# Ced3-han/PepFlowww

Measured on AMD Instinct MI355X. Metric: residues x denoise-steps / s, higher is better.
Workload: dtype f32 (fp32 storage and accumulation; matrix products as 3 x f16 split MFMA, ~22-bit operands); 1 GPU; cfg4/GPU: B=64 x 128-residue synthetic pockets (112 ctx + 16 gen) per GPU; per_gpu_batch=64, residues=128, global_batch=64, parallelism=batch-shard x1, hipgraph=True, precision=fp32

## Files before the change

pepflowww_amd/csrc/common.h:

```cpp
#pragma once
#include <hip/hip_runtime.h>

static inline int pf_cu_count() {
    static int cache[64] = {0};
    int dev = 0, c = 256;
    if (hipGetDevice(&dev) != hipSuccess) return 256;
    if (dev >= 0 && dev < 64 && cache[dev] > 0) return cache[dev];
    if (hipDeviceGetAttribute(&c, hipDeviceAttributeMultiprocessorCount, dev) != hipSuccess || c <= 0) c = 256;
    if (dev >= 0 && dev < 64) cache[dev] = c;
    return c;
}
#include <stdint.h>

#define PF_WAVE 64

typedef float f32x4 __attribute__((ext_vector_type(4)));

__device__ __forceinline__ f32x4 mfma16(float a, float b, f32x4 c) {
    return __builtin_amdgcn_mfma_f32_16x16x4f32(a, b, c, 0, 0, 0);
}

__device__ __forceinline__ void lds_barrier() {
    asm volatile("s_waitcnt lgkmcnt(0)" ::: "memory");
    __builtin_amdgcn_s_barrier();
    asm volatile("" ::: "memory");
}

template <int CTRL, int BANK = 0xF>
__device__ __forceinline__ float dpp_mov(float old, float v) {
    return __int_as_float(__builtin_amdgcn_update_dpp(__float_as_int(old), __float_as_int(v), CTRL, 0xF, BANK, false));
}
__device__ __forceinline__ float lane_xor1(float v) { return dpp_mov<0xB1>(v, v); }
__device__ __forceinline__ float lane_xor2(float v) { return dpp_mov<0x4E>(v, v); }
__device__ __forceinline__ float lane_xor4(float v) {
    float t = dpp_mov<0x104, 0x5>(v, v);
    return dpp_mov<0x114, 0xA>(t, v);
}
__device__ __forceinline__ float lane_xor8(float v) { return dpp_mov<0x128>(v, v); }
template <int OFF> __device__ __forceinline__ float lane_xor(float v) {
    if constexpr (OFF == 1) return lane_xor1(v);
    else if constexpr (OFF == 2) return lane_xor2(v);
    else if constexpr (OFF == 4) return lane_xor4(v);
    else return lane_xor8(v);
}
__device__ __forceinline__ float sum_xor16(float v) {
    auto r = __builtin_amdgcn_permlane16_swap(__float_as_uint(v), __float_as_uint(v), false, false);
    return __uint_as_float(r[0]) + __uint_as_float(r[1]);
}
__device__ __forceinline__ float sum_xor32(float v) {
    auto r = __builtin_amdgcn_permlane32_swap(__float_as_uint(v), __float_as_uint(v), false, false);
    return __uint_as_float(r[0]) + __uint_as_float(r[1]);
}
__device__ __forceinline__ float max_xor16(float v) {
    auto r = __builtin_amdgcn_permlane16_swap(__float_as_uint(v), __float_as_uint(v), false, false);
    return fmaxf(__uint_as_float(r[0]), __uint_as_float(r[1]));
}
__device__ __forceinline__ float max_xor32(float v) {
    auto r = __builtin_amdgcn_permlane32_swap(__float_as_uint(v), __float_as_uint(v), false, false);
    return fmaxf(__uint_as_float(r[0]), __uint_as_float(r[1]));
}
__device__ __forceinline__ bool pf_rows_all_masked(const int* __restrict__ key_end, int L, int m0, int n, int M) {
    if (!key_end) return false;
    const int mend = m0 + n < M ? m0 + n : M;
    int m = m0;
    while (m < mend) {
        const int b = m / L, i = m - b * L;
        if (i < key_end[b]) return false;
        m = (b + 1) * L;
    }
    return true;
}
__device__ __forceinline__ float row16_sum(float v) {
    v += lane_xor8(v); v += lane_xor4(v); v += lane_xor2(v); v += lane_xor1(v);
    return v;
}
__device__ __forceinline__ float row16_max(float v) {
    v = fmaxf(v, lane_xor8(v)); v = fmaxf(v, lane_xor4(v)); v = fmaxf(v, lane_xor2(v)); v = fmaxf(v, lane_xor1(v));
    return v;
}
__device__ __forceinline__ float wave_sum(float v) { return sum_xor32(sum_xor16(row16_sum(v))); }
__device__ __forceinline__ float wave_max(float v) { return max_xor32(max_xor16(row16_max(v))); }

__device__ __forceinline__ float keep_if(bool ok, float v) { return __uint_as_float(__float_as_uint(v) & (ok ? 0xffffffffu : 0u)); }
__device__ __forceinline__ float4 keep_if(bool ok, const float4& v) {
    const unsigned m = ok ? 0xffffffffu : 0u;
    return make_float4(__uint_as_float(__float_as_uint(v.x) & m), __uint_as_float(__float_as_uint(v.y) & m),
                       __uint_as_float(__float_as_uint(v.z) & m), __uint_as_float(__float_as_uint(v.w) & m));
}

template <int MT, int NT>
__device__ __forceinline__ void mfma_slice(const float4 (&a)[MT], const float4 (&b)[NT], f32x4 (&acc)[MT][NT]) {
#pragma unroll
    for (int mt = 0; mt < MT; ++mt)
#pragma unroll
        for (int nt = 0; nt < NT; ++nt) {
            acc[mt][nt] = mfma16(a[mt].x, b[nt].x, acc[mt][nt]);
            acc[mt][nt] = mfma16(a[mt].y, b[nt].y, acc[mt][nt]);
            acc[mt][nt] = mfma16(a[mt].z, b[nt].z, acc[mt][nt]);
            acc[mt][nt] = mfma16(a[mt].w, b[nt].w, acc[mt][nt]);
        }
}

template <int NT, int PF_DEPTH = 4>
struct BStream {
    const float* wrow[NT];
    bool wok[NT];
    float4 ring[PF_DEPTH][NT];
    int nslices;

    __device__ __forceinline__ void init(const float* __restrict__ W, int ldw, int n0, int n_valid, int K) {
        const int lane = threadIdx.x & 63;
        const int r = lane & 15, g = lane >> 4;
        nslices = K >> 4;
#pragma unroll
        for (int nt = 0; nt < NT; ++nt) {
            const int n = n0 + 16 * nt + r;
            wok[nt] = n < n_valid;
            wrow[nt] = W + (size_t)(wok[nt] ? n : 0) * ldw + 4 * g;
        }
    }
    __device__ __forceinline__ void load(int slot_static, int slice, float4 (&dst)[NT]) {
        (void)slot_static;
#pragma unroll
        for (int nt = 0; nt < NT; ++nt)
            dst[nt] = *reinterpret_cast<const float4*>(wrow[nt] + 16 * slice);
    }
    __device__ __forceinline__ void prefetch() {
#pragma unroll
        for (int d = 0; d < PF_DEPTH; ++d)
            if (d < nslices) load(d, d, ring[d]);
    }
};

template <int MT, int NT, int PF_DEPTH>
__device__ __forceinline__ void gemm_ldsA_stream(const float* __restrict__ A_lds, int lda, BStream<NT, PF_DEPTH>& bs,
                                                 f32x4 (&acc)[MT][NT], int slice0, int count) {
    const int lane = threadIdx.x & 63;
    const float* arow = A_lds + (lane & 15) * lda + 4 * (lane >> 4);
    const int ns = bs.nslices;
    for (int base = 0; base < count; base += PF_DEPTH) {
#pragma unroll
        for (int u = 0; u < PF_DEPTH; ++u) {
            if (base + u < count) {
                const int sl = slice0 + base + u;
                float4 a[MT];
#pragma unroll
                for (int mt = 0; mt < MT; ++mt)
                    a[mt] = *reinterpret_cast<const float4*>(arow + mt * 16 * lda + 16 * (base + u));
                mfma_slice<MT, NT>(a, bs.ring[u], acc);
                if (sl + PF_DEPTH < ns) bs.load(u, sl + PF_DEPTH, bs.ring[u]);
            }
        }
    }
}

template <int MT, int NT>
__device__ __forceinline__ void gemm_ldsA_glbB(const float* __restrict__ A_lds, int lda,
                                               const float* __restrict__ W, int ldw, int n0, int n_valid,
                                               int K, f32x4 (&acc)[MT][NT]) {
    BStream<NT> bs;
    bs.init(W, ldw, n0, n_valid, K);
    bs.prefetch();
    gemm_ldsA_stream<MT, NT, 4>(A_lds, lda, bs, acc, 0, bs.nslices);
}

typedef _Float16 half8 __attribute__((ext_vector_type(8)));
typedef _Float16 half4 __attribute__((ext_vector_type(4)));
__device__ __forceinline__ float exp_softmax(float x) { return __builtin_amdgcn_exp2f(x * 1.4426950408889634f); }
constexpr float PF_LO_SCALE = 2048.f, PF_LO_INV = 1.f / 2048.f;

__device__ __forceinline__ f32x4 mfma_h(half8 a, half8 b, f32x4 c) {
    return __builtin_amdgcn_mfma_f32_16x16x32_f16(a, b, c, 0, 0, 0);
}
constexpr float PF_F16_MAX = 65504.f;
#ifndef PF_SPLIT_SATURATE
#define PF_SPLIT_SATURATE 1
#endif
__device__ __forceinline__ void split4(const float (&v)[4], half4& hi, half4& lo) {
#pragma unroll
    for (int e = 0; e < 4; ++e) {
#if PF_SPLIT_SATURATE
        const float vc = fminf(fmaxf(v[e], -PF_F16_MAX), PF_F16_MAX) + v[e] * 0.f;
#else
        const float vc = v[e];
#endif
        const _Float16 h = (_Float16)vc;
        hi[e] = h;
        lo[e] = (_Float16)__builtin_fmaf((float)h, -PF_LO_SCALE, vc * PF_LO_SCALE);
    }
}
__device__ __forceinline__ float join(f32x4 m, f32x4 c, int e) { return m[e] + c[e] * PF_LO_INV; }

template <class V> __device__ __forceinline__ void pf_pin(V& v) { asm("" : "+v"(v)); }

__device__ __forceinline__ void pf_kfrag_put(_Float16* kf, int i, int t8, int g, const float (&v)[4]) {
    half4 hi, lo;
#pragma unroll
    for (int e = 0; e < 4; ++e) hi[e] = (_Float16)v[e];
    pf_pin(hi);
#pragma unroll
    for (int e = 0; e < 4; ++e) lo[e] = (_Float16)(v[e] - (float)hi[e]);
    _Float16* d = kf + (size_t)(i >> 4) * 4096 + (t8 >> 1) * 1024 + ((i & 15) + 16 * g) * 8 + (t8 & 1) * 4;
    *reinterpret_cast<half4*>(d) = hi;
    *reinterpret_cast<half4*>(d + 512) = lo;
}
constexpr int PF_KFRAG_TILE_B = 8192;

template <int WT, int D, bool SP = false>
struct WSplit {
    const _Float16* wh[WT];
    const _Float16* wl[WT];
    half8 rh[D][WT], rl[D][WT];
    int nsteps;
    __device__ __forceinline__ void init(const void* planes, int Npad, int K, int n0) {
        const int lane = threadIdx.x & 63;
        const _Float16* hi = reinterpret_cast<const _Float16*>(planes);
        const _Float16* lo = hi + (size_t)Npad * K;
        nsteps = K >> 5;
#pragma unroll
        for (int wt = 0; wt < WT; ++wt) {
            const size_t off = ((size_t)((n0 >> 4) + wt) * nsteps * 64 + lane) * 8;
            wh[wt] = hi + off;
            wl[wt] = lo + off;
        }
    }
    __device__ __forceinline__ void load(int step, half8 (&dh)[WT], half8 (&dl)[WT]) {
#pragma unroll
        for (int wt = 0; wt < WT; ++wt) {
            dh[wt] = *reinterpret_cast<const half8*>(wh[wt] + (size_t)step * 512);
            if constexpr (!SP) dl[wt] = *reinterpret_cast<const half8*>(wl[wt] + (size_t)step * 512);
        }
    }
    __device__ __forceinline__ void prefetch() {
#pragma unroll
        for (int d = 0; d < D; ++d)
            if (d < nsteps) load(d, rh[d], rl[d]);
    }
};

template <int WT, int D, bool SP>
__device__ __forceinline__ void gemm_split16(WSplit<WT, D, SP>& ws, const _Float16* Xh, const _Float16* Xl, int ldx,
                                             f32x4 (&am)[WT], f32x4 (&ac)[WT], int step0, int count) {
    const int lane = threadIdx.x & 63;
    const int off = (lane & 15) * ldx + 8 * (lane >> 4);
    for (int base = 0; base < count; base += D) {
#pragma unroll
        for (int u = 0; u < D; ++u) {
            if (base + u < count) {
                const int st = step0 + base + u;
                const half8 xh = *reinterpret_cast<const half8*>(Xh + off + 32 * (base + u));
                half8 xl;
                if constexpr (!SP) xl = *reinterpret_cast<const half8*>(Xl + off + 32 * (base + u));
#pragma unroll
                for (int wt = 0; wt < WT; ++wt) {
                    am[wt] = mfma_h(ws.rh[u][wt], xh, am[wt]);
                    if constexpr (!SP) {
                        ac[wt] = mfma_h(ws.rh[u][wt], xl, ac[wt]);
                        ac[wt] = mfma_h(ws.rl[u][wt], xh, ac[wt]);
                    }
                }
                if (st + D < ws.nsteps) ws.load(st + D, ws.rh[u], ws.rl[u]);
            }
        }
    }
}
template <int WT, int D, bool SP, int RT>
__device__ __forceinline__ void gemm_split16r(WSplit<WT, D, SP>& ws, const _Float16* Xh, const _Float16* Xl, int ldx,
                                              f32x4 (&am)[RT][WT], f32x4 (&ac)[RT][WT], int step0, int count) {
    const int lane = threadIdx.x & 63;
    const int off = (lane & 15) * ldx + 8 * (lane >> 4);
    for (int base = 0; base < count; base += D) {
#pragma unroll
        for (int u = 0; u < D; ++u) {
            if (base + u < count) {
                const int st = step0 + base + u;
#pragma unroll
                for (int rt = 0; rt < RT; ++rt) {
                    const half8 xh = *reinterpret_cast<const half8*>(Xh + rt * 16 * ldx + off + 32 * (base + u));
                    half8 xl;
                    if constexpr (!SP) xl = *reinterpret_cast<const half8*>(Xl + rt * 16 * ldx + off + 32 * (base + u));
#pragma unroll
                    for (int wt = 0; wt < WT; ++wt) {
                        am[rt][wt] = mfma_h(ws.rh[u][wt], xh, am[rt][wt]);
                        if constexpr (!SP) {
                            ac[rt][wt] = mfma_h(ws.rh[u][wt], xl, ac[rt][wt]);
                            ac[rt][wt] = mfma_h(ws.rl[u][wt], xh, ac[rt][wt]);
                        }
                    }
                }
                if (st + D < ws.nsteps) ws.load(st + D, ws.rh[u], ws.rl[u]);
            }
        }
    }
}
template <int WT> __device__ __forceinline__ void acc_zero1(f32x4 (&a)[WT], f32x4 (&b)[WT]) {
#pragma unroll
    for (int wt = 0; wt < WT; ++wt) { a[wt] = (f32x4){0.f, 0.f, 0.f, 0.f}; b[wt] = (f32x4){0.f, 0.f, 0.f, 0.f}; }
}

template <int WT>
struct WPre {
    half8 h[WT], l[WT];
    __device__ __forceinline__ void load(const void* planes, int N, int Kw, int n0) {
        const int lane = threadIdx.x & 63;
        const int wsteps = Kw >> 5;
        const _Float16* wh = reinterpret_cast<const _Float16*>(planes) + ((size_t)(n0 >> 4) * wsteps * 64 + lane) * 8;
        const _Float16* wl = wh + (size_t)N * Kw;
        const size_t tstride = (size_t)wsteps * 512;
#pragma unroll
        for (int wt = 0; wt < WT; ++wt) {
            h[wt] = *reinterpret_cast<const half8*>(wh + wt * tstride);
            l[wt] = *reinterpret_cast<const half8*>(wl + wt * tstride);
        }
    }
};

template <int WT, int PT, bool SP = false>
__device__ __forceinline__ void gemm_split_lowreg(const void* planes, int N, int Kw, int n0, int K,
                                                  const _Float16* Xh, const _Float16* Xl, int ldx,
                                                  f32x4 (&am)[WT][PT], f32x4 (&ac)[WT][PT]) {
    static_assert(PT % 2 == 0, "row tiles are fed in pairs");
    const int lane = threadIdx.x & 63, r = lane & 15, g = lane >> 4;
    const int wsteps = Kw >> 5, nst = K >> 5;
    const _Float16* wh = reinterpret_cast<const _Float16*>(planes) + ((size_t)(n0 >> 4) * wsteps * 64 + lane) * 8;
    const _Float16* wl = wh + (size_t)N * Kw;
    const size_t tstride = (size_t)wsteps * 512;
    const _Float16* xh = Xh + r * ldx + 8 * g;
    const _Float16* xl = Xl + r * ldx + 8 * g;
    for (int st = 0; st < nst; ++st) {
        half8 bh[WT], bl[WT];
#pragma unroll
        for (int wt = 0; wt < WT; ++wt) {
            bh[wt] = *reinterpret_cast<const half8*>(wh + wt * tstride + (size_t)st * 512);
            if constexpr (!SP) bl[wt] = *reinterpret_cast<const half8*>(wl + wt * tstride + (size_t)st * 512);
        }
#pragma unroll
        for (int p0 = 0; p0 < PT; p0 += 2) {
            half8 ah[2], al[2];
#pragma unroll
            for (int q = 0; q < 2; ++q) {
                ah[q] = *reinterpret_cast<const half8*>(xh + (p0 + q) * 16 * ldx + 32 * st);
                if constexpr (!SP) al[q] = *reinterpret_cast<const half8*>(xl + (p0 + q) * 16 * ldx + 32 * st);
            }
#pragma unroll
            for (int wt = 0; wt < WT; ++wt)
#pragma unroll
                for (int q = 0; q < 2; ++q) am[wt][p0 + q] = mfma_h(bh[wt], ah[q], am[wt][p0 + q]);
            if constexpr (!SP) {
#pragma unroll
                for (int wt = 0; wt < WT; ++wt)
#pragma unroll
                    for (int q = 0; q < 2; ++q) ac[wt][p0 + q] = mfma_h(bh[wt], al[q], ac[wt][p0 + q]);
#pragma unroll
                for (int wt = 0; wt < WT; ++wt)
#pragma unroll
                    for (int q = 0; q < 2; ++q) ac[wt][p0 + q] = mfma_h(bl[wt], ah[q], ac[wt][p0 + q]);
            }
        }
    }
}

template <int WT, int PT, bool SWZ = false, bool SP = false, bool SWAP = false>
__device__ __forceinline__ void gemm_split(const void* planes, int N, int Kw, int n0, int K,
                                           const _Float16* Xh, const _Float16* Xl, int ldx,
                                           f32x4 (&am)[WT][PT], f32x4 (&ac)[WT][PT], const WPre<WT>* pre = nullptr) {
    const int lane = threadIdx.x & 63, r = lane & 15, g = lane >> 4;
    const int wsteps = Kw >> 5;
    const _Float16* wh = reinterpret_cast<const _Float16*>(planes) + ((size_t)(n0 >> 4) * wsteps * 64 + lane) * 8;
    const _Float16* wl = wh + (size_t)N * Kw;
    const size_t tstride = (size_t)wsteps * 512;
    const int gs = SWZ ? (g ^ ((r >> 2) & 1)) : g;
    const _Float16* xh = Xh + r * ldx + 8 * gs;
    const _Float16* xl = Xl + r * ldx + 8 * gs;
    half8 bh[WT], bl[WT], nh[WT], nl[WT];
#pragma unroll
    for (int wt = 0; wt < WT; ++wt) {
        if (pre) { bh[wt] = pre->h[wt]; bl[wt] = pre->l[wt]; }
        else {
            bh[wt] = *reinterpret_cast<const half8*>(wh + wt * tstride);
            if constexpr (!SP) bl[wt] = *reinterpret_cast<const half8*>(wl + wt * tstride);
        }
    }
    const int nst = K >> 5;
    for (int st = 0; st < nst; ++st) {
        if (st + 1 < nst) {
#pragma unroll
            for (int wt = 0; wt < WT; ++wt) {
                nh[wt] = *reinterpret_cast<const half8*>(wh + wt * tstride + (size_t)(st + 1) * 512);
                if constexpr (!SP) nl[wt] = *reinterpret_cast<const half8*>(wl + wt * tstride + (size_t)(st + 1) * 512);
            }
        }
        half8 ah[PT], al[PT];
#pragma unroll
        for (int pt = 0; pt < PT; ++pt) {
            ah[pt] = *reinterpret_cast<const half8*>(xh + pt * 16 * ldx + 32 * st);
            if constexpr (!SP) al[pt] = *reinterpret_cast<const half8*>(xl + pt * 16 * ldx + 32 * st);
        }
#pragma unroll
        for (int wt = 0; wt < WT; ++wt)
#pragma unroll
            for (int pt = 0; pt < PT; ++pt) am[wt][pt] = SWAP ? mfma_h(ah[pt], bh[wt], am[wt][pt]) : mfma_h(bh[wt], ah[pt], am[wt][pt]);
        if constexpr (!SP) {
#pragma unroll
            for (int wt = 0; wt < WT; ++wt)
#pragma unroll
                for (int pt = 0; pt < PT; ++pt) ac[wt][pt] = SWAP ? mfma_h(al[pt], bh[wt], ac[wt][pt]) : mfma_h(bh[wt], al[pt], ac[wt][pt]);
#pragma unroll
            for (int wt = 0; wt < WT; ++wt)
#pragma unroll
                for (int pt = 0; pt < PT; ++pt) ac[wt][pt] = SWAP ? mfma_h(ah[pt], bl[wt], ac[wt][pt]) : mfma_h(bl[wt], ah[pt], ac[wt][pt]);
        }
#pragma unroll
        for (int wt = 0; wt < WT; ++wt) { bh[wt] = nh[wt]; if constexpr (!SP) bl[wt] = nl[wt]; }
    }
}

__device__ __forceinline__ int swz_col(int n0, int r, int g) {
    return n0 + 8 * ((g >> 1) ^ ((r >> 2) & 1)) + 4 * (g & 1);
}

template <int MT, int NT>
__device__ __forceinline__ void acc_zero(f32x4 (&acc)[MT][NT]) {
#pragma unroll
    for (int mt = 0; mt < MT; ++mt)
#pragma unroll
        for (int nt = 0; nt < NT; ++nt) acc[mt][nt] = (f32x4){0.f, 0.f, 0.f, 0.f};
}

__device__ __forceinline__ int xcd_remap(int bid, int nblk) {
    const int q = nblk >> 3, rem = nblk & 7, x = bid & 7, k = bid >> 3;
    return (x < rem ? x * (q + 1) : rem * (q + 1) + (x - rem) * q) + k;
}

#define PF_CHECK_LAUNCH() do { hipError_t e_ = hipGetLastError(); if (e_ != hipSuccess) return (int)e_; } while (0)

struct PfOncePerDevice {
    bool done[32] = {};
    bool first() {
        int d = 0;
        (void)hipGetDevice(&d);
        d &= 31;
        if (done[d]) return false;
        done[d] = true;
        return true;
    }
};
```

pepflowww_amd/csrc/node_track.hip:

```cpp
#include "common.h"
#include "rigid_dev.h"
#include "../../include/pepflow_hip.h"

#ifdef PF_PROFILE
__device__ long long g_prof[64];
#ifndef PF_PROF_LAST
#define PF_PROF_LAST 1
#endif
#define PROF(i) do { if (LAST == (PF_PROF_LAST != 0) && blockIdx.x == 0 && threadIdx.x == 0) g_prof[i] = clock64(); } while (0)
extern "C" int pf_debug_prof(long long* out, int n) {
    return (int)hipMemcpyFromSymbol(out, HIP_SYMBOL(g_prof), sizeof(long long) * n, 0, hipMemcpyDeviceToHost);
}
#else
#define PROF(i)
#endif

namespace {

constexpr int TR = 16;
constexpr int LDX = 132;
constexpr int LDP = 136;
constexpr int NTHR = 512;
#ifndef PF_NT_MINW
#define PF_NT_MINW 2
#endif

struct Planes { _Float16* h; _Float16* l; };

struct LnParams { float g[8], b[8]; };
__device__ __forceinline__ void ln_load(LnParams& p, const float* __restrict__ g, const float* __restrict__ b) {
    const int sub = threadIdx.x & 15;
    const float4 g0 = *reinterpret_cast<const float4*>(g + 8 * sub), g1 = *reinterpret_cast<const float4*>(g + 8 * sub + 4);
    const float4 b0 = *reinterpret_cast<const float4*>(b + 8 * sub), b1 = *reinterpret_cast<const float4*>(b + 8 * sub + 4);
    p.g[0] = g0.x; p.g[1] = g0.y; p.g[2] = g0.z; p.g[3] = g0.w; p.g[4] = g1.x; p.g[5] = g1.y; p.g[6] = g1.z; p.g[7] = g1.w;
    p.b[0] = b0.x; p.b[1] = b0.y; p.b[2] = b0.z; p.b[3] = b0.w; p.b[4] = b1.x; p.b[5] = b1.y; p.b[6] = b1.z; p.b[7] = b1.w;
}
template <int ROWS = 16, bool KFR = false>
__device__ __forceinline__ void ln_tile(float* T, const LnParams& p, float mk, Planes out, int m0, int M, float* gout, _Float16* kf = nullptr, int i0 = 0) {
    const int tid = threadIdx.x;
    if (tid < 16 * ROWS) {
        const int row = tid >> 4, sub = tid & 15, m = m0 + row;
        float v[8];
        {
            const float4 a = *reinterpret_cast<const float4*>(T + row * LDX + 8 * sub);
            const float4 b = *reinterpret_cast<const float4*>(T + row * LDX + 8 * sub + 4);
            v[0] = a.x; v[1] = a.y; v[2] = a.z; v[3] = a.w; v[4] = b.x; v[5] = b.y; v[6] = b.z; v[7] = b.w;
        }
        float s = ((v[0] + v[1]) + (v[2] + v[3])) + ((v[4] + v[5]) + (v[6] + v[7]));
        s = row16_sum(s);
        const float mean = s / 128.f;
        float q = 0.f;
#pragma unroll
        for (int c = 0; c < 8; ++c) { const float d = v[c] - mean; q += d * d; }
        q = row16_sum(q);
        const float rstd = rsqrtf(q / 128.f + 1e-5f);
        float y[8];
#pragma unroll
        for (int c = 0; c < 8; ++c) y[c] = ((v[c] - mean) * rstd * p.g[c] + p.b[c]) * mk;
        *reinterpret_cast<float4*>(T + row * LDX + 8 * sub) = make_float4(y[0], y[1], y[2], y[3]);
        *reinterpret_cast<float4*>(T + row * LDX + 8 * sub + 4) = make_float4(y[4], y[5], y[6], y[7]);
        half4 h0, l0, h1, l1;
        const float y0[4] = {y[0], y[1], y[2], y[3]}, y1[4] = {y[4], y[5], y[6], y[7]};
        split4(y0, h0, l0);
        split4(y1, h1, l1);
        *reinterpret_cast<half4*>(out.h + row * LDP + 8 * sub) = h0;
        *reinterpret_cast<half4*>(out.h + row * LDP + 8 * sub + 4) = h1;
        *reinterpret_cast<half4*>(out.l + row * LDP + 8 * sub) = l0;
        *reinterpret_cast<half4*>(out.l + row * LDP + 8 * sub + 4) = l1;
        if (gout && m < M) {
            *reinterpret_cast<float4*>(gout + (size_t)m * 128 + 8 * sub) = make_float4(y[0], y[1], y[2], y[3]);
            *reinterpret_cast<float4*>(gout + (size_t)m * 128 + 8 * sub + 4) = make_float4(y[4], y[5], y[6], y[7]);
        }
        if constexpr (KFR) {
            if (kf && m < M) {
                pf_kfrag_put(kf, i0 + row, sub >> 1, 2 * (sub & 1), y0);
                pf_kfrag_put(kf, i0 + row, sub >> 1, 2 * (sub & 1) + 1, y1);
            }
        }
    }
}

__device__ __forceinline__ float4 sel4(bool ok, const float4& v) {
    const float f = ok ? 1.f : 0.f;
    return make_float4(v.x * f, v.y * f, v.z * f, v.w * f);
}

__device__ __forceinline__ void put_planes(Planes p, int r, int n, const float (&v)[4]) {
    half4 hi, lo;
    split4(v, hi, lo);
    *reinterpret_cast<half4*>(p.h + r * LDP + n) = hi;
    *reinterpret_cast<half4*>(p.l + r * LDP + n) = lo;
}

template <bool SP, bool DUMP = false, bool PM = false>
__global__ __launch_bounds__(NTHR, PF_NT_MINW) void node_head_kernel(pf_node_head_args a) {
    extern __shared__ __attribute__((aligned(16))) unsigned char smem_raw[];
    constexpr int CK = 256, LDC = CK + 8;
    _Float16* Ch = reinterpret_cast<_Float16*>(smem_raw);
    float* X = reinterpret_cast<float*>(smem_raw + 2 * 2 * TR * LDC * sizeof(_Float16));
    Planes Xa = {reinterpret_cast<_Float16*>(X + TR * LDX), reinterpret_cast<_Float16*>(X + TR * LDX) + TR * LDP};
    const int tid = threadIdx.x, wave = tid >> 6, lane = tid & 63;
    const int r = lane & 15, g = lane >> 4;
    const int m0 = blockIdx.x * TR, M = a.rows;
    if (pf_rows_all_masked(a.key_end, a.key_L, m0, TR, M)) return;
    const int n = wave * 16 + 4 * g;

    constexpr int C0 = PM ? 4 : 0;
    WSplit<1, 8, SP> ws;
    ws.init(a.w_out_f16, 128, PF_IPA_FEATS - C0 * 256, wave * 16);
    ws.prefetch();
    LnParams lnp;
    ln_load(lnp, a.ln_g, a.ln_b);
    const float4 bias_out = *reinterpret_cast<const float4*>(a.b_out + n);
    float4 bias_in[3];
#pragma unroll
    for (int wt = 0; wt < 3; ++wt) bias_in[wt] = *reinterpret_cast<const float4*>(a.b_in + wave * 48 + wt * 16 + 4 * g);
    const int mr = m0 + r;
    const int mrc = mr < M ? mr : M - 1;
    const float rmask_ld = a.mask[mrc];
    const float4 rres_ld = *reinterpret_cast<const float4*>(a.s_in + (size_t)mrc * 128 + n);
    const int srow = tid >> 5, sc4 = tid & 31;
    const bool sok = m0 + srow < M;
    const float* src = a.feats + (size_t)(sok ? m0 + srow : 0) * PF_IPA_FEATS + 4 * sc4;
    constexpr int NCH = PF_IPA_FEATS / CK;
    float4 st[NCH][2];
#pragma unroll
    for (int c = 0; c < NCH; ++c)
#pragma unroll
        for (int hlf = 0; hlf < 2; ++hlf)
            st[c][hlf] = *reinterpret_cast<const float4*>(src + c * CK + hlf * 128);
    auto commit = [&](int c) {
        _Float16* bh = Ch + (c & 1) * 2 * TR * LDC;
        _Float16* bl = bh + TR * LDC;
#pragma unroll
        for (int hlf = 0; hlf < 2; ++hlf) {
            const float4 sv = sel4(sok, st[c][hlf]);
            const float v[4] = {sv.x, sv.y, sv.z, sv.w};
            half4 hi, lo;
            split4(v, hi, lo);
            *reinterpret_cast<half4*>(bh + srow * LDC + hlf * 128 + 4 * sc4) = hi;
            *reinterpret_cast<half4*>(bl + srow * LDC + hlf * 128 + 4 * sc4) = lo;
        }
    };
    if constexpr (PM) {
        auto add4 = [](const float4& p, const float4& q) { return make_float4(p.x + q.x, p.y + q.y, p.z + q.z, p.w + q.w); };
        float4 ev = sel4(sok, st[0][0]), od = sel4(sok, st[0][1]);
#pragma unroll
        for (int c = 1; c < 4; ++c) { ev = add4(ev, sel4(sok, st[c][0])); od = add4(od, sel4(sok, st[c][1])); }
        *reinterpret_cast<float4*>(X + srow * LDX + 4 * sc4) = add4(ev, od);
    }
    commit(C0);
    __syncthreads();
    f32x4 am[1], ac[1];
    acc_zero1<1>(am, ac);
#pragma unroll
    for (int c = C0; c < NCH; ++c) {
        const _Float16* bh = Ch + (c & 1) * 2 * TR * LDC;
        gemm_split16(ws, bh, bh + TR * LDC, LDC, am, ac, (c - C0) * 8, 8);
        if (c + 1 < NCH) commit(c + 1);
        __syncthreads();
    }
    WSplit<3, 4, SP> wq;
    wq.init(a.w_in_f16, 384, 128, wave * 48);
    wq.prefetch();
    {
        const float rmask = rmask_ld * (mr < M ? 1.f : 0.f);
        const float4 rres = sel4(mr < M, rres_ld);
        float4 hs = make_float4(0.f, 0.f, 0.f, 0.f);
        if constexpr (PM) hs = *reinterpret_cast<const float4*>(X + r * LDX + n);
        auto lin = [&](int e, float h) { const float j = join(am[0], ac[0], e); if constexpr (PM) return j + h; else return j; };
        float4 y;
        y.x = (lin(0, hs.x) + bias_out.x) * rmask + rres.x;
        y.y = (lin(1, hs.y) + bias_out.y) * rmask + rres.y;
        y.z = (lin(2, hs.z) + bias_out.z) * rmask + rres.z;
        y.w = (lin(3, hs.w) + bias_out.w) * rmask + rres.w;
        *reinterpret_cast<float4*>(X + r * LDX + n) = y;
        if constexpr (DUMP) { if (mr < M) *reinterpret_cast<float4*>(a.dump_a0 + (size_t)mr * 128 + n) = y; }
    }
    __syncthreads();
    ln_tile(X, lnp, 1.f, Xa, m0, M, a.s_ipa);
    __syncthreads();
    f32x4 qm[3], qc[3];
    acc_zero1<3>(qm, qc);
    gemm_split16(wq, Xa.h, Xa.l, LDP, qm, qc, 0, 4);
    if (mr < M) {
#pragma unroll
        for (int wt = 0; wt < 3; ++wt) {
            float4 y;
            y.x = join(qm[wt], qc[wt], 0) + bias_in[wt].x; y.y = join(qm[wt], qc[wt], 1) + bias_in[wt].y;
            y.z = join(qm[wt], qc[wt], 2) + bias_in[wt].z; y.w = join(qm[wt], qc[wt], 3) + bias_in[wt].w;
            *reinterpret_cast<float4*>(a.qkv + (size_t)mr * 384 + wave * 48 + wt * 16 + 4 * g) = y;
        }
    }
}

constexpr int TR2 = 32;
template <bool SP, bool PM = false>
__global__ __launch_bounds__(NTHR, PF_NT_MINW) void node_head32_kernel(pf_node_head_args a) {
    extern __shared__ __attribute__((aligned(16))) unsigned char smem_raw[];
    constexpr int CK = 256, LDC = CK + 8;
    _Float16* Ch = reinterpret_cast<_Float16*>(smem_raw);
    float* X = reinterpret_cast<float*>(smem_raw + 2 * 2 * TR2 * LDC * sizeof(_Float16));
    Planes Xa = {reinterpret_cast<_Float16*>(X + TR2 * LDX), reinterpret_cast<_Float16*>(X + TR2 * LDX) + TR2 * LDP};
    const int tid = threadIdx.x, wave = tid >> 6, lane = tid & 63;
    const int r = lane & 15, g = lane >> 4;
    int m0 = blockIdx.x * TR2, M = a.rows;
    if (a.key_end) {
        const int tps = (a.key_L + TR2 - 1) / TR2, b = blockIdx.x / tps, i0 = (blockIdx.x - b * tps) * TR2;
        if (i0 >= a.key_end[b]) return;
        m0 = b * a.key_L + i0;
        M = (b + 1) * a.key_L;
    }
    const int n = wave * 16 + 4 * g;

    constexpr int C0 = PM ? 4 : 0;
    WSplit<1, 8, SP> ws;
    ws.init(a.w_out_f16, 128, PF_IPA_FEATS - C0 * 256, wave * 16);
    ws.prefetch();
    LnParams lnp;
    ln_load(lnp, a.ln_g, a.ln_b);
    const float4 bias_out = *reinterpret_cast<const float4*>(a.b_out + n);
    float4 bias_in[3];
#pragma unroll
    for (int wt = 0; wt < 3; ++wt) bias_in[wt] = *reinterpret_cast<const float4*>(a.b_in + wave * 48 + wt * 16 + 4 * g);
    float rmask_ld[2];
    float4 rres_ld[2];
#pragma unroll
    for (int rt = 0; rt < 2; ++rt) {
        const int mr = m0 + rt * 16 + r;
        const int mrc = mr < M ? mr : M - 1;
        rmask_ld[rt] = a.mask[mrc];
        rres_ld[rt] = *reinterpret_cast<const float4*>(a.s_in + (size_t)mrc * 128 + n);
    }
    constexpr int NCH = PF_IPA_FEATS / CK;
    float4 st[2][4];
    auto fetch = [&](int c, float4 (&d)[4]) {
#pragma unroll
        for (int u = 0; u < 4; ++u) {
            const int idx = tid + u * NTHR, row = idx >> 6, c4 = idx & 63;
            const int m = m0 + row < M ? m0 + row : M - 1;
            d[u] = *reinterpret_cast<const float4*>(a.feats + (size_t)m * PF_IPA_FEATS + c * CK + 4 * c4);
        }
    };
    auto commit = [&](int c, const float4 (&d)[4]) {
        _Float16* bh = Ch + (c & 1) * 2 * TR2 * LDC;
        _Float16* bl = bh + TR2 * LDC;
#pragma unroll
        for (int u = 0; u < 4; ++u) {
            const int idx = tid + u * NTHR, row = idx >> 6, c4 = idx & 63;
            const float4 sv = sel4(m0 + row < M, d[u]);
            const float v[4] = {sv.x, sv.y, sv.z, sv.w};
            half4 hi, lo;
            split4(v, hi, lo);
            *reinterpret_cast<half4*>(bh + row * LDC + 4 * c4) = hi;
            *reinterpret_cast<half4*>(bl + row * LDC + 4 * c4) = lo;
        }
    };
    fetch(0, st[0]);
    fetch(1, st[1]);
    if constexpr (PM) {
        auto add4 = [](const float4& p, const float4& q) { return make_float4(p.x + q.x, p.y + q.y, p.z + q.z, p.w + q.w); };
        float4 hsum[4];
#pragma unroll
        for (int c = 0; c < 4; ++c) {
#pragma unroll
            for (int u = 0; u < 4; ++u) {
                const int idx = tid + u * NTHR, row = idx >> 6;
                const float4 v = sel4(m0 + row < M, st[c & 1][u]);
                hsum[u] = c == 0 ? v : add4(hsum[u], v);
            }
            fetch(c + 2, st[c & 1]);
        }
#pragma unroll
        for (int u = 0; u < 4; ++u) {
            const int idx = tid + u * NTHR, row = idx >> 6, c4 = idx & 63;
            float4 o;
            o.x = __shfl_xor(hsum[u].x, 32); o.y = __shfl_xor(hsum[u].y, 32); o.z = __shfl_xor(hsum[u].z, 32); o.w = __shfl_xor(hsum[u].w, 32);
            if (c4 < 32) *reinterpret_cast<float4*>(X + row * LDX + 4 * c4) = add4(hsum[u], o);
        }
    }
    commit(C0, st[C0 & 1]);
    __syncthreads();
    f32x4 am[2][1], ac[2][1];
#pragma unroll
    for (int rt = 0; rt < 2; ++rt) acc_zero1<1>(am[rt], ac[rt]);
#pragma unroll
    for (int c = C0; c < NCH; ++c) {
        if (!PM && c + 2 < NCH) fetch(c + 2, st[c & 1]);
        const _Float16* bh = Ch + (c & 1) * 2 * TR2 * LDC;
        gemm_split16r<1, 8, SP, 2>(ws, bh, bh + TR2 * LDC, LDC, am, ac, (c - C0) * 8, 8);
        if (c + 1 < NCH) commit(c + 1, st[(c + 1) & 1]);
        __syncthreads();
    }
    WSplit<3, 4, SP> wq;
    wq.init(a.w_in_f16, 384, 128, wave * 48);
    wq.prefetch();
#pragma unroll
    for (int rt = 0; rt < 2; ++rt) {
        const int mr = m0 + rt * 16 + r;
        const float rmask = rmask_ld[rt] * (mr < M ? 1.f : 0.f);
        const float4 rres = sel4(mr < M, rres_ld[rt]);
        float4 hs = make_float4(0.f, 0.f, 0.f, 0.f);
        if constexpr (PM) hs = *reinterpret_cast<const float4*>(X + (rt * 16 + r) * LDX + n);
        auto lin = [&](int e, float h) { const float j = join(am[rt][0], ac[rt][0], e); if constexpr (PM) return j + h; else return j; };
        float4 y;
        y.x = (lin(0, hs.x) + bias_out.x) * rmask + rres.x;
        y.y = (lin(1, hs.y) + bias_out.y) * rmask + rres.y;
        y.z = (lin(2, hs.z) + bias_out.z) * rmask + rres.z;
        y.w = (lin(3, hs.w) + bias_out.w) * rmask + rres.w;
        *reinterpret_cast<float4*>(X + (rt * 16 + r) * LDX + n) = y;
    }
    __syncthreads();
    ln_tile<TR2>(X, lnp, 1.f, Xa, m0, M, a.s_ipa);
    __syncthreads();
    f32x4 qm[2][3], qc[2][3];
#pragma unroll
    for (int rt = 0; rt < 2; ++rt) acc_zero1<3>(qm[rt], qc[rt]);
    gemm_split16r<3, 4, SP, 2>(wq, Xa.h, Xa.l, LDP, qm, qc, 0, 4);
#pragma unroll
    for (int rt = 0; rt < 2; ++rt) {
        const int mr = m0 + rt * 16 + r;
        if (mr < M) {
#pragma unroll
            for (int wt = 0; wt < 3; ++wt) {
                float4 y;
                y.x = join(qm[rt][wt], qc[rt][wt], 0) + bias_in[wt].x; y.y = join(qm[rt][wt], qc[rt][wt], 1) + bias_in[wt].y;
                y.z = join(qm[rt][wt], qc[rt][wt], 2) + bias_in[wt].z; y.w = join(qm[rt][wt], qc[rt][wt], 3) + bias_in[wt].w;
                *reinterpret_cast<float4*>(a.qkv + (size_t)mr * 384 + wave * 48 + wt * 16 + 4 * g) = y;
            }
        }
    }
}

template <bool LAST, bool SP, int RT, bool DUMP = false>
__global__ __launch_bounds__(NTHR, PF_NT_MINW) void node_tfmr_kernel(pf_node_tfmr_args a, int LP, int LDS_S) {
    constexpr int TR = 16 * RT;
    extern __shared__ __attribute__((aligned(16))) float smem[];
    float* T0 = smem;
    float* T1 = T0 + TR * LDX;
    float* U = T1 + TR * LDX;
    _Float16* pl = reinterpret_cast<_Float16*>(U + TR * 8);
    Planes Xa = {pl, pl + TR * LDP}, Xb = {pl + 2 * TR * LDP, pl + 3 * TR * LDP};
    float* S = reinterpret_cast<float*>(pl + 4 * TR * LDP);
    const int tid = threadIdx.x, wave = tid >> 6, lane = tid & 63;
    const int r = lane & 15, g = lane >> 4;
    const int L = a.L;
    const int tiles = (L + TR - 1) / TR;
    const int lid = a.key_end ? (int)blockIdx.x : xcd_remap(blockIdx.x, gridDim.x);
    const int b = lid / tiles;
    const int i0 = (lid - b * tiles) * TR;
    const size_t rowb = (size_t)b * L;
    if (a.key_end && i0 >= __builtin_amdgcn_readfirstlane(a.key_end[b])) return;
    if constexpr (LAST) {
        if (a.row_on) {
            int any = 0;
#pragma unroll
            for (int rt = 0; rt < RT; ++rt) any |= a.row_on[((int)rowb + min(i0 + 16 * rt, L - 16)) >> 4];
            if (!__builtin_amdgcn_readfirstlane(any)) return;
        }
    }
    const int m0 = (int)rowb + i0;
    const int M = (int)rowb + L;
    const int n = wave * 16 + 4 * g;
    int mr[RT];
#pragma unroll
    for (int rt = 0; rt < RT; ++rt) mr[rt] = m0 + 16 * rt + r;
    auto dump4 = [&](float* p, int rt, float x, float y, float z, float w) {
        if constexpr (DUMP) { if (mr[rt] < M) *reinterpret_cast<float4*>(p + (size_t)mr[rt] * 128 + n) = make_float4(x, y, z, w); }
    };

    PROF(0);
    const int h = wave & 3;
    float4 q0[RT], q1[RT];
#pragma unroll
    for (int rt = 0; rt < RT; ++rt) {
        const int i = i0 + 16 * rt + r;
        const float* qrow = a.qkv + (rowb + (i < L ? i : 0)) * 384 + h * 32 + 4 * g;
        q0[rt] = *reinterpret_cast<const float4*>(qrow);
        q1[rt] = *reinterpret_cast<const float4*>(qrow + 16);
    }
    const float4 z4 = make_float4(0.f, 0.f, 0.f, 0.f);
    const int par = wave >> 2;
    auto kload = [&](int j0, float4 (&k0)[2], float4 (&k1)[2], float (&km)[2]) {
#pragma unroll
        for (int t = 0; t < 2; ++t) {
            const int j = j0 + 32 * t + r;
            const int jc = j < L ? j : L - 1;
            const float* krow = a.qkv + (rowb + jc) * 384 + 128 + h * 32 + 4 * g;
            k0[t] = *reinterpret_cast<const float4*>(krow);
            k1[t] = *reinterpret_cast<const float4*>(krow + 16);
            km[t] = a.mask[rowb + jc];
        }
    };
    float4 kfA0[2], kfA1[2], kfB0[2], kfB1[2];
    float kfAm[2], kfBm[2];
    kload(16 * par, kfA0, kfA1, kfAm);
    kload(16 * par + 64, kfB0, kfB1, kfBm);
    asm volatile("" ::: "memory");
    const int ct = wave >> 2;
    const float* vcol = a.qkv + rowb * 384 + 256 + h * 32 + ct * 16 + r;
    auto vload = [&](int k0, float (&vb)[4][4]) {
#pragma unroll
        for (int s4 = 0; s4 < 4; ++s4)
#pragma unroll
            for (int t = 0; t < 4; ++t) {
                int j = k0 + 16 * s4 + 4 * g + t;
                j = j < L ? j : L - 1;
                vb[s4][t] = vcol[(size_t)j * 384];
            }
    };
    float vbA[4][4], vbB[4][4];
    vload(0, vbA);
    vload(64, vbB);
    asm volatile("" ::: "memory");
    WSplit<1, 4, SP> ws;
    ws.init(a.w_o_f16, 128, 128, wave * 16);
    ws.prefetch();
    LnParams ln1, ln2, ln3;
    ln_load(ln1, a.n1_g, a.n1_b);
    ln_load(ln2, a.n2_g, a.n2_b);
    if (LAST) ln_load(ln3, a.nt_g, a.nt_b);
    const float4 bias_o = *reinterpret_cast<const float4*>(a.b_o + n), bias_1 = *reinterpret_cast<const float4*>(a.b_1 + n),
                 bias_2 = *reinterpret_cast<const float4*>(a.b_2 + n);
    float4 bias_post = z4, bias_t1 = z4, bias_t2 = z4, bias_t3 = z4, bias_bb = z4, bias_init = z4;
    float4 bias_in[3] = {z4, z4, z4}, bias_pre[4] = {z4, z4, z4, z4};
    float4 rres_ld[RT], rsipa_ld[RT];
#pragma unroll
    for (int rt = 0; rt < RT; ++rt) {
        const int mrc = mr[rt] < M ? mr[rt] : M - 1;
        rres_ld[rt] = *reinterpret_cast<const float4*>(a.resid + (size_t)mrc * 128 + n);
        rsipa_ld[rt] = LAST ? *reinterpret_cast<const float4*>(a.s_ipa + (size_t)mrc * 128 + n) : z4;
    }
    float lnmask_ld = 1.f;
    const int lnrow = m0 + ((tid & (16 * TR - 1)) >> 4);
    auto load_tail_consts = [&]() {
        bias_post = *reinterpret_cast<const float4*>(a.b_post + n);
        bias_t1 = *reinterpret_cast<const float4*>(a.b_t1 + n);
        bias_t2 = *reinterpret_cast<const float4*>(a.b_t2 + n);
        bias_t3 = *reinterpret_cast<const float4*>(a.b_t3 + n);
        bias_bb = *reinterpret_cast<const float4*>(a.b_bb + 4 * (g & 1));
        if (a.has_et) {
            bias_init = *reinterpret_cast<const float4*>(a.b_init + (wave & 3) * 16 + 4 * g);
#pragma unroll
            for (int wt = 0; wt < 4; ++wt) bias_pre[wt] = *reinterpret_cast<const float4*>(a.b_pre + wave * 64 + wt * 16 + 4 * g);
        }
        lnmask_ld = a.mask[lnrow < M ? lnrow : M - 1];
    };
    if (LAST) {
        if (RT == 1) load_tail_consts();
    } else {
#pragma unroll
        for (int wt = 0; wt < 3; ++wt) bias_in[wt] = *reinterpret_cast<const float4*>(a.b_in_next + wave * 48 + wt * 16 + 4 * g);
    }

    PROF(1);
    {
        const float scale = 0.17677669529663687f;
        auto score_block = [&](int j0, const float4 (&k0)[2], const float4 (&k1)[2], const float (&km)[2]) {
#pragma unroll
            for (int t = 0; t < 2; ++t) {
                const int j = j0 + 32 * t + r;
                if (j0 + 32 * t < LP) {
                    const bool keep = j < L && km[t] > 0.5f;
#pragma unroll
                    for (int rt = 0; rt < RT; ++rt) {
                        f32x4 acc = {0.f, 0.f, 0.f, 0.f};
                        acc = mfma16(q0[rt].x, k0[t].x, acc); acc = mfma16(q0[rt].y, k0[t].y, acc); acc = mfma16(q0[rt].z, k0[t].z, acc); acc = mfma16(q0[rt].w, k0[t].w, acc);
                        acc = mfma16(q1[rt].x, k1[t].x, acc); acc = mfma16(q1[rt].y, k1[t].y, acc); acc = mfma16(q1[rt].z, k1[t].z, acc); acc = mfma16(q1[rt].w, k1[t].w, acc);
#pragma unroll
                        for (int e = 0; e < 4; ++e) S[((16 * rt + 4 * g + e) * 4 + h) * LDS_S + j] = keep ? acc[e] * scale : -3.0e38f;
                    }
                }
            }
        };
        score_block(16 * par, kfA0, kfA1, kfAm);
        if (16 * par + 64 < LP) score_block(16 * par + 64, kfB0, kfB1, kfBm);
        for (int j0 = 16 * par + 128; j0 < LP; j0 += 64) {
            float4 kn0[2], kn1[2];
            float knm[2];
            kload(j0, kn0, kn1, knm);
            score_block(j0, kn0, kn1, knm);
        }
    }
    __syncthreads();
    PROF(2);
#pragma unroll
    for (int ps = 0; ps < RT; ++ps) {
        const int sub = lane & 7;
        float* sp = S + ((ps * 8 + wave) * 8 + (lane >> 3)) * LDS_S;
        if (LP <= 256) {
            float4 v[8];
#pragma unroll
            for (int u = 0; u < 8; ++u) {
                const int j = 4 * sub + 32 * u;
                v[u] = j < LP ? *reinterpret_cast<const float4*>(sp + j) : make_float4(-3.0e38f, -3.0e38f, -3.0e38f, -3.0e38f);
            }
            float m = -3.0e38f;
#pragma unroll
            for (int u = 0; u < 8; ++u) m = fmaxf(m, fmaxf(fmaxf(v[u].x, v[u].y), fmaxf(v[u].z, v[u].w)));
            m = fmaxf(m, lane_xor1(m)); m = fmaxf(m, lane_xor2(m)); m = fmaxf(m, lane_xor4(m));
            float sum = 0.f;
#pragma unroll
            for (int u = 0; u < 8; ++u) {
                v[u].x = (v[u].x > -1.0e38f) ? exp_softmax(v[u].x - m) : 0.f; v[u].y = (v[u].y > -1.0e38f) ? exp_softmax(v[u].y - m) : 0.f;
                v[u].z = (v[u].z > -1.0e38f) ? exp_softmax(v[u].z - m) : 0.f; v[u].w = (v[u].w > -1.0e38f) ? exp_softmax(v[u].w - m) : 0.f;
                sum += (v[u].x + v[u].y) + (v[u].z + v[u].w);
            }
            sum += lane_xor1(sum); sum += lane_xor2(sum); sum += lane_xor4(sum);
            const float inv = 1.f / sum;
#pragma unroll
            for (int u = 0; u < 8; ++u) {
                const int j = 4 * sub + 32 * u;
                if (j < LP) *reinterpret_cast<float4*>(sp + j) = make_float4(v[u].x * inv, v[u].y * inv, v[u].z * inv, v[u].w * inv);
            }
        } else {
            float m = -3.0e38f;
            for (int j = sub; j < LP; j += 8) m = fmaxf(m, sp[j]);
            m = fmaxf(m, lane_xor1(m)); m = fmaxf(m, lane_xor2(m)); m = fmaxf(m, lane_xor4(m));
            float sum = 0.f;
            for (int j = sub; j < LP; j += 8) { const float e = (sp[j] > -1.0e38f) ? exp_softmax(sp[j] - m) : 0.f; sp[j] = e; sum += e; }
            sum += lane_xor1(sum); sum += lane_xor2(sum); sum += lane_xor4(sum);
            const float inv = 1.f / sum;
            for (int j = sub; j < LP; j += 8) sp[j] *= inv;
        }
    }
    __syncthreads();
    PROF(3);
    {
        f32x4 acc[RT];
#pragma unroll
        for (int rt = 0; rt < RT; ++rt) acc[rt] = (f32x4){0.f, 0.f, 0.f, 0.f};
        const float* prow = S + (r * 4 + h) * LDS_S + 4 * g;
        auto pv_block = [&](int k0, const float (&vb)[4][4]) {
#pragma unroll
            for (int s4 = 0; s4 < 4; ++s4) {
                if (k0 + 16 * s4 < LP) {
#pragma unroll
                    for (int rt = 0; rt < RT; ++rt) {
                        const float4 pa = *reinterpret_cast<const float4*>(prow + rt * 64 * LDS_S + k0 + 16 * s4);
                        acc[rt] = mfma16(pa.x, vb[s4][0], acc[rt]); acc[rt] = mfma16(pa.y, vb[s4][1], acc[rt]);
                        acc[rt] = mfma16(pa.z, vb[s4][2], acc[rt]); acc[rt] = mfma16(pa.w, vb[s4][3], acc[rt]);
                    }
                }
            }
        };
        pv_block(0, vbA);
        if (64 < LP) pv_block(64, vbB);
        for (int k0 = 128; k0 < LP; k0 += 64) {
            float vn[4][4];
            vload(k0, vn);
            pv_block(k0, vn);
        }
        const int col = h * 32 + ct * 16 + r;
#pragma unroll
        for (int rt = 0; rt < RT; ++rt)
#pragma unroll
            for (int e = 0; e < 4; ++e) {
                const _Float16 hi = (_Float16)acc[rt][e];
                Xa.h[(16 * rt + 4 * g + e) * LDP + col] = hi;
                Xa.l[(16 * rt + 4 * g + e) * LDP + col] = (_Float16)((acc[rt][e] - (float)hi) * PF_LO_SCALE);
                if constexpr (DUMP) { if (m0 + 16 * rt + 4 * g + e < M) a.dump[0][(size_t)(m0 + 16 * rt + 4 * g + e) * 128 + col] = acc[rt][e]; }
            }
    }
    if (LAST && RT == 2) load_tail_consts();
    __syncthreads();
    PROF(4);

    f32x4 am[RT][1], ac[RT][1];
    auto zero = [&]() {
#pragma unroll
        for (int rt = 0; rt < RT; ++rt) acc_zero1<1>(am[rt], ac[rt]);
    };
    auto joined = [&](int rt, const float4& bias, float (&v)[4]) {
        v[0] = join(am[rt][0], ac[rt][0], 0) + bias.x; v[1] = join(am[rt][0], ac[rt][0], 1) + bias.y;
        v[2] = join(am[rt][0], ac[rt][0], 2) + bias.z; v[3] = join(am[rt][0], ac[rt][0], 3) + bias.w;
    };
    auto relu4 = [](float (&v)[4]) {
#pragma unroll
        for (int e = 0; e < 4; ++e) v[e] = fmaxf(v[e], 0.f);
    };
    zero();
    gemm_split16r<1, 4, SP, RT>(ws, Xa.h, Xa.l, LDP, am, ac, 0, 4);
    ws.init(a.w_1_f16, 128, 128, wave * 16);
    ws.prefetch();
#pragma unroll
    for (int rt = 0; rt < RT; ++rt) {
        const float4 rres = sel4(mr[rt] < M, rres_ld[rt]);
        float v[4];
        joined(rt, bias_o, v);
        *reinterpret_cast<float4*>(T1 + (16 * rt + r) * LDX + n) = make_float4(v[0] + rres.x, v[1] + rres.y, v[2] + rres.z, v[3] + rres.w);
        dump4(a.dump[1], rt, v[0] + rres.x, v[1] + rres.y, v[2] + rres.z, v[3] + rres.w);
    }
    __syncthreads();
    ln_tile<TR>(T1, ln1, 1.f, Xb, m0, M, DUMP ? a.dump[2] : nullptr);
    __syncthreads();
    PROF(5);
    zero();
    gemm_split16r<1, 4, SP, RT>(ws, Xb.h, Xb.l, LDP, am, ac, 0, 4);
    ws.init(a.w_2_f16, 128, 128, wave * 16);
    ws.prefetch();
#pragma unroll
    for (int rt = 0; rt < RT; ++rt) {
        float v[4];
        joined(rt, bias_1, v);
        relu4(v);
        put_planes(Xa, 16 * rt + r, n, v);
        dump4(a.dump[3], rt, v[0], v[1], v[2], v[3]);
    }
    __syncthreads();
    PROF(6);
    zero();
    gemm_split16r<1, 4, SP, RT>(ws, Xa.h, Xa.l, LDP, am, ac, 0, 4);
    auto lin2_to_t0 = [&]() {
#pragma unroll
        for (int rt = 0; rt < RT; ++rt) {
            const float4 u = *reinterpret_cast<const float4*>(T1 + (16 * rt + r) * LDX + n);
            float v[4];
            joined(rt, bias_2, v);
            *reinterpret_cast<float4*>(T0 + (16 * rt + r) * LDX + n) = make_float4(v[0] + u.x, v[1] + u.y, v[2] + u.z, v[3] + u.w);
            dump4(a.dump[4], rt, v[0] + u.x, v[1] + u.y, v[2] + u.z, v[3] + u.w);
        }
    };
    if constexpr (!LAST) {
        WSplit<3, 4, SP> wq;
        wq.init(a.w_in_next_f16, 384, 128, wave * 48);
        wq.prefetch();
        lin2_to_t0();
        __syncthreads();
        ln_tile<TR>(T0, ln2, 1.f, Xb, m0, M, a.v_out);
        __syncthreads();
        PROF(7);
        f32x4 qm[RT][3], qc[RT][3];
#pragma unroll
        for (int rt = 0; rt < RT; ++rt) acc_zero1<3>(qm[rt], qc[rt]);
        gemm_split16r<3, 4, SP, RT>(wq, Xb.h, Xb.l, LDP, qm, qc, 0, 4);
#pragma unroll
        for (int rt = 0; rt < RT; ++rt) {
            if (mr[rt] < M) {
#pragma unroll
                for (int wt = 0; wt < 3; ++wt) {
                    float4 y;
                    y.x = join(qm[rt][wt], qc[rt][wt], 0) + bias_in[wt].x; y.y = join(qm[rt][wt], qc[rt][wt], 1) + bias_in[wt].y;
                    y.z = join(qm[rt][wt], qc[rt][wt], 2) + bias_in[wt].z; y.w = join(qm[rt][wt], qc[rt][wt], 3) + bias_in[wt].w;
                    *reinterpret_cast<float4*>(a.qkv_out + (size_t)mr[rt] * 384 + wave * 48 + wt * 16 + 4 * g) = y;
                }
            }
        }
        PROF(8);
    } else {
        ws.init(a.w_post_f16, 128, 128, wave * 16);
        ws.prefetch();
        lin2_to_t0();
        float4 fq = make_float4(1.f, 0.f, 0.f, 0.f);
        float fR[9], fx[3], fmask = 0.f;
        if (tid < TR && m0 + tid < M) {
            const int m = m0 + tid;
            fq = *reinterpret_cast<const float4*>(a.quat_in + (size_t)m * 4);
#pragma unroll
            for (int k = 0; k < 9; ++k) fR[k] = a.rot_in[(size_t)m * 9 + k];
#pragma unroll
            for (int k = 0; k < 3; ++k) fx[k] = a.trans_in[(size_t)m * 3 + k];
            fmask = a.mask[m];
        }
        __syncthreads();
        ln_tile<TR>(T0, ln2, 1.f, Xb, m0, M, DUMP ? a.dump[5] : nullptr);
        __syncthreads();
        PROF(7);
        zero();
        gemm_split16r<1, 4, SP, RT>(ws, Xb.h, Xb.l, LDP, am, ac, 0, 4);
        ws.init(a.w_t1_f16, 128, 128, wave * 16);
        ws.prefetch();
#pragma unroll
        for (int rt = 0; rt < RT; ++rt) {
            const float4 rsipa = sel4(mr[rt] < M, rsipa_ld[rt]);
            float v[4];
            joined(rt, bias_post, v);
            v[0] += rsipa.x; v[1] += rsipa.y; v[2] += rsipa.z; v[3] += rsipa.w;
            *reinterpret_cast<float4*>(T1 + (16 * rt + r) * LDX + n) = make_float4(v[0], v[1], v[2], v[3]);
            put_planes(Xa, 16 * rt + r, n, v);
            dump4(a.dump[6], rt, v[0], v[1], v[2], v[3]);
        }
        __syncthreads();
        PROF(8);
        zero();
        gemm_split16r<1, 4, SP, RT>(ws, Xa.h, Xa.l, LDP, am, ac, 0, 4);
        ws.init(a.w_t2_f16, 128, 128, wave * 16);
        ws.prefetch();
#pragma unroll
        for (int rt = 0; rt < RT; ++rt) {
            float v[4];
            joined(rt, bias_t1, v);
            relu4(v);
            put_planes(Xb, 16 * rt + r, n, v);
            dump4(a.dump[7], rt, v[0], v[1], v[2], v[3]);
        }
        __syncthreads();
        zero();
        gemm_split16r<1, 4, SP, RT>(ws, Xb.h, Xb.l, LDP, am, ac, 0, 4);
        ws.init(a.w_t3_f16, 128, 128, wave * 16);
        ws.prefetch();
#pragma unroll
        for (int rt = 0; rt < RT; ++rt) {
            float v[4];
            joined(rt, bias_t2, v);
            relu4(v);
            put_planes(Xa, 16 * rt + r, n, v);
            dump4(a.dump[8], rt, v[0], v[1], v[2], v[3]);
        }
        __syncthreads();
        zero();
        gemm_split16r<1, 4, SP, RT>(ws, Xa.h, Xa.l, LDP, am, ac, 0, 4);
        const bool do_bb = wave == 0, do_init = a.has_et && wave >= 4;
        if (do_bb) { ws.init(a.w_bb_f16, 16, 128, 0); ws.prefetch(); }
        else if (do_init) { ws.init(a.w_init_f16, 64, 128, (wave - 4) * 16); ws.prefetch(); }
        WSplit<4, 2, SP> wp;
        if (a.has_et) { wp.init(a.w_pre_f16, PF_ET_PRE, 64, wave * 64); wp.prefetch(); }
#pragma unroll
        for (int rt = 0; rt < RT; ++rt) {
            const float4 s0 = *reinterpret_cast<const float4*>(T1 + (16 * rt + r) * LDX + n);
            float v[4];
            joined(rt, bias_t3, v);
            *reinterpret_cast<float4*>(T0 + (16 * rt + r) * LDX + n) = make_float4(v[0] + s0.x, v[1] + s0.y, v[2] + s0.z, v[3] + s0.w);
            dump4(a.dump[9], rt, v[0] + s0.x, v[1] + s0.y, v[2] + s0.z, v[3] + s0.w);
        }
        __syncthreads();
        _Float16* kfs = DUMP || !a.k_frag_s ? nullptr : reinterpret_cast<_Float16*>(a.k_frag_s) + (size_t)b * ((L + 15) >> 4) * (PF_KFRAG_TILE_B / 2);
        ln_tile<TR, !DUMP>(T0, ln3, lnmask_ld * (lnrow < M ? 1.f : 0.f), Xb, m0, M, a.s_out, kfs, i0);
        __syncthreads();
        PROF(9);
        if (do_bb || do_init) {
            zero();
            gemm_split16r<1, 4, SP, RT>(ws, Xb.h, Xb.l, LDP, am, ac, 0, 4);
#pragma unroll
            for (int rt = 0; rt < RT; ++rt) {
                float v[4];
                if (do_bb) {
                    joined(rt, bias_bb, v);
                    if (g < 2) *reinterpret_cast<float4*>(U + (16 * rt + r) * 8 + 4 * g) = make_float4(v[0], v[1], v[2], v[3]);
                    if constexpr (DUMP) { if (g < 2 && mr[rt] < M) *reinterpret_cast<float4*>(a.dump[10] + (size_t)mr[rt] * 8 + 4 * g) = make_float4(v[0], v[1], v[2], v[3]); }
                } else {
                    joined(rt, bias_init, v);
                    put_planes(Xa, 16 * rt + r, (wave - 4) * 16 + 4 * g, v);
                }
            }
        }
        __syncthreads();
        if (tid < TR && m0 + tid < M) {
            const int m = m0 + tid;
            float Ro[9], xo[3];
            float4 qo;
            rigid_update_dev(fq, fR, fx, U + tid * 8, fmask, qo, Ro, xo);
            *reinterpret_cast<float4*>(a.quat_out + (size_t)m * 4) = qo;
#pragma unroll
            for (int k = 0; k < 3; ++k) a.trans_out[(size_t)m * 3 + k] = xo[k];
#pragma unroll
            for (int k = 0; k < 9; ++k) a.rot_out[(size_t)m * 9 + k] = Ro[k];
        }
        PROF(10);
        if (a.has_et) {
            f32x4 pm[RT][4], pc[RT][4];
#pragma unroll
            for (int rt = 0; rt < RT; ++rt) acc_zero1<4>(pm[rt], pc[rt]);
            PROF(12);
            gemm_split16r<4, 2, SP, RT>(wp, Xa.h, Xa.l, LDP, pm, pc, 0, 2);
            PROF(13);
#pragma unroll
            for (int rt = 0; rt < RT; ++rt) {
                if (mr[rt] < M) {
#pragma unroll
                    for (int wt = 0; wt < 4; ++wt) {
                        float4 y;
                        y.x = join(pm[rt][wt], pc[rt][wt], 0) + bias_pre[wt].x; y.y = join(pm[rt][wt], pc[rt][wt], 1) + bias_pre[wt].y;
                        y.z = join(pm[rt][wt], pc[rt][wt], 2) + bias_pre[wt].z; y.w = join(pm[rt][wt], pc[rt][wt], 3) + bias_pre[wt].w;
                        *reinterpret_cast<float4*>(a.pre + (size_t)mr[rt] * PF_ET_PRE + wave * 64 + wt * 16 + 4 * g) = y;
                    }
                }
            }
        } else if (a.logits_out) {
            __syncthreads();
            Planes Xc = {reinterpret_cast<_Float16*>(T0), reinterpret_cast<_Float16*>(T0) + TR * LDP};
#pragma unroll
            for (int net = 0; net < 2; ++net) {
                const int nout = net ? 5 : 20, ntile = net ? 1 : 2;
                ws.init(a.h_w[net][0], 128, 128, wave * 16);
                ws.prefetch();
                const float4 hb0 = *reinterpret_cast<const float4*>(a.h_b[net][0] + n), hb1 = *reinterpret_cast<const float4*>(a.h_b[net][1] + n);
                zero();
                gemm_split16r<1, 4, SP, RT>(ws, Xb.h, Xb.l, LDP, am, ac, 0, 4);
                ws.init(a.h_w[net][1], 128, 128, wave * 16);
                ws.prefetch();
#pragma unroll
                for (int rt = 0; rt < RT; ++rt) {
                    float v[4];
                    joined(rt, hb0, v);
                    relu4(v);
                    put_planes(Xa, 16 * rt + r, n, v);
                }
                __syncthreads();
                zero();
                gemm_split16r<1, 4, SP, RT>(ws, Xa.h, Xa.l, LDP, am, ac, 0, 4);
                if (wave < ntile) { ws.init(a.h_w[net][2], 16 * ntile, 128, wave * 16); ws.prefetch(); }
#pragma unroll
                for (int rt = 0; rt < RT; ++rt) {
                    float v[4];
                    joined(rt, hb1, v);
                    relu4(v);
                    put_planes(Xc, 16 * rt + r, n, v);
                }
                __syncthreads();
                if (wave < ntile) {
                    const float4 hb2 = *reinterpret_cast<const float4*>(a.h_b[net][2] + n);
                    zero();
                    gemm_split16r<1, 4, SP, RT>(ws, Xc.h, Xc.l, LDP, am, ac, 0, 4);
#pragma unroll
                    for (int rt = 0; rt < RT; ++rt) {
                        if (mr[rt] < M) {
                            float* op = (net ? a.ang_out : a.logits_out) + (size_t)mr[rt] * nout;
                            float v[4];
                            joined(rt, hb2, v);
#pragma unroll
                            for (int e = 0; e < 4; ++e)
                                if (n + e < nout) op[n + e] = v[e];
                        }
                    }
                }
                __syncthreads();
            }
        }
        PROF(11);
    }
}

constexpr int LDF = 640 + 8;
template <bool SP>
__global__ __launch_bounds__(NTHR) void input_mixer_kernel(pf_input_mixer_args a) {
    extern __shared__ __attribute__((aligned(16))) unsigned char smem_raw[];
    Planes Xf = {reinterpret_cast<_Float16*>(smem_raw), reinterpret_cast<_Float16*>(smem_raw) + TR * LDF};
    Planes Xa = {Xf.l + TR * LDF, Xf.l + TR * LDF + TR * LDP};
    const int tid = threadIdx.x, wave = tid >> 6, lane = tid & 63;
    const int r = lane & 15, g = lane >> 4;
    const int m0 = blockIdx.x * TR, M = a.B * a.L;
    const int n = wave * 16 + 4 * g;
    WSplit<1, 8, SP> w0;
    w0.init(a.w0_f16, 128, 640, wave * 16);
    w0.prefetch();
    const float4 b0 = *reinterpret_cast<const float4*>(a.b0 + n);
    const float4 b2 = *reinterpret_cast<const float4*>(a.b2 + n);
    const int mr = m0 + r, mrc = mr < M ? mr : M - 1;
    const float rmask = a.mask[mrc] * (mr < M ? 1.f : 0.f);
    __shared__ float TC[2][128];
    const int b_first = m0 / a.L, b_last = min(m0 + TR - 1, M - 1) / a.L;
    const bool tc_shared = b_last - b_first < 2;
    if (tc_shared && tid < 128 * (b_last - b_first + 1)) {
        const int bi = tid >> 7, k = tid & 127;
        const float tt = a.t[b_first + bi] * 2056.f;
        TC[bi][k] = k < 64 ? sinf(tt * a.time_freq[k]) : cosf(tt * a.time_freq[k - 64]);
    }
    __syncthreads();
    for (int idx = tid; idx < TR * 160; idx += NTHR) {
        const int row = idx / 160, c4 = idx - row * 160;
        const int m = min(m0 + row, M - 1);
        const int b = m / a.L;
        float v[4];
        if (c4 < 32) {
            const float4 t = *reinterpret_cast<const float4*>(a.node_embed + (size_t)m * 128 + 4 * c4);
            v[0] = t.x; v[1] = t.y; v[2] = t.z; v[3] = t.w;
        } else if (c4 < 64) {
            long long sq = a.seqs[m];
            sq = sq < 0 ? 0 : (sq > 21 ? 21 : sq);
            const float4 t = *reinterpret_cast<const float4*>(a.seq_table + sq * 128 + 4 * (c4 - 32));
            v[0] = t.x; v[1] = t.y; v[2] = t.z; v[3] = t.w;
        } else {
            const float tt = a.t[b] * 2056.f;
#pragma unroll
            for (int e = 0; e < 4; ++e) {
                const int c = 4 * c4 + e;
                float x;
                if (c < 384 && tc_shared) x = TC[b - b_first][c - 256];
                else if (c < 320) x = sinf(tt * a.time_freq[c - 256]);
                else if (c < 384) x = cosf(tt * a.time_freq[c - 320]);
                else if (c < 629) {
                    const int q = c - 384, d = q / 49, k = q - d * 49;
                    const float ang = a.angles[(size_t)m * 5 + d];
                    if (k == 0) x = ang;
                    else if (k < 25) x = sinf(ang * a.ang_freq[k - 1]);
                    else x = cosf(ang * a.ang_freq[k - 25]);
                } else x = 0.f;
                v[e] = x;
            }
        }
        half4 hi, lo;
        split4(v, hi, lo);
        *reinterpret_cast<half4*>(Xf.h + row * LDF + 4 * c4) = hi;
        *reinterpret_cast<half4*>(Xf.l + row * LDF + 4 * c4) = lo;
    }
    if (tid < TR && m0 + tid < M) {
        float R[9], q[4];
#pragma unroll
        for (int k = 0; k < 9; ++k) R[k] = a.rot[(size_t)(m0 + tid) * 9 + k];
        rot_to_quat_dev(R, q);
        *reinterpret_cast<float4*>(a.quat + (size_t)(m0 + tid) * 4) = make_float4(q[0], q[1], q[2], q[3]);
    }
    __syncthreads();
    f32x4 am[1], ac[1];
    acc_zero1<1>(am, ac);
    gemm_split16(w0, Xf.h, Xf.l, LDF, am, ac, 0, 20);
    WSplit<1, 4, SP> w2;
    w2.init(a.w2_f16, 128, 128, wave * 16);
    w2.prefetch();
    {
        const float v[4] = {fmaxf(join(am[0], ac[0], 0) + b0.x, 0.f), fmaxf(join(am[0], ac[0], 1) + b0.y, 0.f),
                            fmaxf(join(am[0], ac[0], 2) + b0.z, 0.f), fmaxf(join(am[0], ac[0], 3) + b0.w, 0.f)};
        put_planes(Xa, r, n, v);
    }
    __syncthreads();
    acc_zero1<1>(am, ac);
    gemm_split16(w2, Xa.h, Xa.l, LDP, am, ac, 0, 4);
    if (mr < M) {
        float4 y;
        y.x = (join(am[0], ac[0], 0) + b2.x) * rmask; y.y = (join(am[0], ac[0], 1) + b2.y) * rmask;
        y.z = (join(am[0], ac[0], 2) + b2.z) * rmask; y.w = (join(am[0], ac[0], 3) + b2.w) * rmask;
        *reinterpret_cast<float4*>(a.s_out + (size_t)mr * 128 + n) = y;
        if (a.k_frag_s) {
            const int b = mr / a.L;
            const float v[4] = {y.x, y.y, y.z, y.w};
            pf_kfrag_put(reinterpret_cast<_Float16*>(a.k_frag_s) + (size_t)b * ((a.L + 15) >> 4) * (PF_KFRAG_TILE_B / 2), mr - b * a.L, wave, g, v);
        }
    }
}

}

extern "C" int pf_input_mixer_fwd(const pf_input_mixer_args* a, pf_stream_t stream) {
    if (!a || !a->node_embed || !a->seq_table || !a->seqs || !a->t || !a->time_freq || !a->ang_freq || !a->angles || !a->w0_f16 ||
        !a->b0 || !a->w2_f16 || !a->b2 || !a->mask || !a->rot || !a->quat || !a->s_out || a->B <= 0 || a->L <= 0)
        return PF_E_BADARG;
    const int rows = a->B * a->L;
    const size_t lds = (size_t)2 * TR * LDF * sizeof(_Float16) + (size_t)2 * TR * LDP * sizeof(_Float16);
    if (a->single_pass) hipLaunchKernelGGL(input_mixer_kernel<true>, dim3((unsigned)((rows + TR - 1) / TR)), dim3(NTHR), lds, (hipStream_t)stream, *a);
    else hipLaunchKernelGGL(input_mixer_kernel<false>, dim3((unsigned)((rows + TR - 1) / TR)), dim3(NTHR), lds, (hipStream_t)stream, *a);
    PF_CHECK_LAUNCH();
    return 0;
}

extern "C" int pf_node_head_fwd(const pf_node_head_args* a, pf_stream_t stream) {
    if (!a || !a->feats || !a->s_in || !a->mask || !a->w_out_f16 || !a->b_out || !a->ln_g || !a->ln_b || !a->w_in_f16 ||
        !a->b_in || !a->s_ipa || !a->qkv || a->rows <= 0)
        return PF_E_BADARG;
    const size_t lds = (size_t)2 * 2 * TR * 264 * sizeof(_Float16) + (size_t)TR * LDX * sizeof(float) +
                       (size_t)2 * TR * LDP * sizeof(_Float16);
    if (a->rows >= pf_cu_count() * TR2 && !a->dump_a0) {
        const size_t lds2 = (size_t)2 * 2 * TR2 * 264 * sizeof(_Float16) + (size_t)TR2 * LDX * sizeof(float) + (size_t)2 * TR2 * LDP * sizeof(_Float16);
        static PfOncePerDevice attr_set;
        if (attr_set.first()) {
            (void)hipFuncSetAttribute((const void*)node_head32_kernel<true>, hipFuncAttributeMaxDynamicSharedMemorySize, 160 * 1024);
            (void)hipFuncSetAttribute((const void*)node_head32_kernel<false>, hipFuncAttributeMaxDynamicSharedMemorySize, 160 * 1024);
            (void)hipFuncSetAttribute((const void*)node_head32_kernel<true, true>, hipFuncAttributeMaxDynamicSharedMemorySize, 160 * 1024);
            (void)hipFuncSetAttribute((const void*)node_head32_kernel<false, true>, hipFuncAttributeMaxDynamicSharedMemorySize, 160 * 1024);
        }
        const bool per_sample = a->key_end && a->key_L > 0 && a->rows % a->key_L == 0;
        pf_node_head_args aa = *a;
        if (!per_sample) aa.key_end = nullptr;
        const dim3 grid(per_sample ? (unsigned)((a->rows / a->key_L) * ((a->key_L + TR2 - 1) / TR2)) : (unsigned)((a->rows + TR2 - 1) / TR2));
        a = &aa;
        if (a->o_premul) {
            if (a->single_pass) hipLaunchKernelGGL((node_head32_kernel<true, true>), grid, dim3(NTHR), lds2, (hipStream_t)stream, *a);
            else hipLaunchKernelGGL((node_head32_kernel<false, true>), grid, dim3(NTHR), lds2, (hipStream_t)stream, *a);
        } else if (a->single_pass) hipLaunchKernelGGL(node_head32_kernel<true>, grid, dim3(NTHR), lds2, (hipStream_t)stream, *a);
        else hipLaunchKernelGGL(node_head32_kernel<false>, grid, dim3(NTHR), lds2, (hipStream_t)stream, *a);
        PF_CHECK_LAUNCH();
        return 0;
    }
    if (a->dump_a0) {
        if (a->single_pass || a->o_premul) return PF_E_BADARG;
        hipLaunchKernelGGL((node_head_kernel<false, true>), dim3((unsigned)((a->rows + TR - 1) / TR)), dim3(NTHR), lds, (hipStream_t)stream, *a);
        PF_CHECK_LAUNCH();
        return 0;
    }
    if (a->o_premul) {
        if (a->single_pass) hipLaunchKernelGGL((node_head_kernel<true, false, true>), dim3((unsigned)((a->rows + TR - 1) / TR)), dim3(NTHR), lds, (hipStream_t)stream, *a);
        else hipLaunchKernelGGL((node_head_kernel<false, false, true>), dim3((unsigned)((a->rows + TR - 1) / TR)), dim3(NTHR), lds, (hipStream_t)stream, *a);
    } else if (a->single_pass) hipLaunchKernelGGL(node_head_kernel<true>, dim3((unsigned)((a->rows + TR - 1) / TR)), dim3(NTHR), lds, (hipStream_t)stream, *a);
    else hipLaunchKernelGGL(node_head_kernel<false>, dim3((unsigned)((a->rows + TR - 1) / TR)), dim3(NTHR), lds, (hipStream_t)stream, *a);
    PF_CHECK_LAUNCH();
    return 0;
}

extern "C" int pf_node_tfmr_fwd(const pf_node_tfmr_args* a, pf_stream_t stream) {
    if (!a || !a->qkv || !a->resid || !a->mask || !a->w_o_f16 || !a->b_o || !a->n1_g || !a->n1_b || !a->w_1_f16 || !a->b_1 ||
        !a->w_2_f16 || !a->b_2 || !a->n2_g || !a->n2_b || a->B <= 0 || a->L <= 0)
        return PF_E_BADARG;
    if (!a->last && (!a->w_in_next_f16 || !a->b_in_next || !a->qkv_out || !a->v_out)) return PF_E_BADARG;
    if (a->last && (!a->s_ipa || !a->w_post_f16 || !a->b_post || !a->w_t1_f16 || !a->b_t1 || !a->w_t2_f16 || !a->b_t2 ||
                    !a->w_t3_f16 || !a->b_t3 || !a->nt_g || !a->nt_b || !a->w_bb_f16 || !a->b_bb || !a->s_out || !a->quat_in ||
                    !a->rot_in || !a->trans_in || !a->quat_out || !a->rot_out || !a->trans_out))
        return PF_E_BADARG;
    if (a->last && a->has_et && (!a->w_init_f16 || !a->b_init || !a->w_pre_f16 || !a->b_pre || !a->pre)) return PF_E_BADARG;
    if (a->last && !a->has_et && a->logits_out) {
        if (!a->ang_out) return PF_E_BADARG;
        for (int net = 0; net < 2; ++net)
            for (int l = 0; l < 3; ++l)
                if (!a->h_w[net][l] || !a->h_b[net][l]) return PF_E_BADARG;
    }
    const int LP = (a->L + 15) / 16 * 16;
    const int LDS_S = LP + 4;
    const int tiles16 = (a->L + 15) / 16;
    auto lds_of = [&](int rt) {
        const int tr = 16 * rt;
        return ((size_t)2 * tr * LDX + tr * 8 + (size_t)tr * 4 * LDS_S) * sizeof(float) + (size_t)4 * tr * LDP * sizeof(_Float16);
    };
    const int RTn = ((long)a->B * tiles16 > pf_cu_count() && a->L > 16 && !a->dump[0] && lds_of(2) <= (size_t)160 * 1024) ? 2 : 1;
    const int TRn = 16 * RTn;
    const size_t lds = lds_of(RTn);
    if (lds > 160 * 1024) return PF_E_TOOLARGE;
    const int tiles = (a->L + TRn - 1) / TRn;
    const dim3 grid((unsigned)(a->B * tiles));
    const int variant = (RTn == 2 ? 4 : 0) + (a->last ? 2 : 0) + (a->single_pass ? 1 : 0);
    static PfOncePerDevice attr_set[8];
#define PF_NT_CASE(V, LASTV, SPV, RTV)                                                                                           \
    case V:                                                                                                                      \
        if (attr_set[V].first()) {                                                                                                      \
            (void)hipFuncSetAttribute((const void*)node_tfmr_kernel<LASTV, SPV, RTV>, hipFuncAttributeMaxDynamicSharedMemorySize, \
                                      160 * 1024);                                                                               \
        }                                                                                                                        \
        hipLaunchKernelGGL((node_tfmr_kernel<LASTV, SPV, RTV>), grid, dim3(NTHR), lds, (hipStream_t)stream, *a, LP, LDS_S);      \
        break;
    if (a->dump[0]) {
        for (int k = 0; k < (a->last ? 11 : 5); ++k)
            if (!a->dump[k]) return PF_E_BADARG;
        if (a->single_pass || RTn != 1) return PF_E_BADARG;
        static PfOncePerDevice dattr[2];
        if (a->last) {
            if (dattr[1].first()) { (void)hipFuncSetAttribute((const void*)node_tfmr_kernel<true, false, 1, true>, hipFuncAttributeMaxDynamicSharedMemorySize, 160 * 1024); }
            hipLaunchKernelGGL((node_tfmr_kernel<true, false, 1, true>), grid, dim3(NTHR), lds, (hipStream_t)stream, *a, LP, LDS_S);
        } else {
            if (dattr[0].first()) { (void)hipFuncSetAttribute((const void*)node_tfmr_kernel<false, false, 1, true>, hipFuncAttributeMaxDynamicSharedMemorySize, 160 * 1024); }
            hipLaunchKernelGGL((node_tfmr_kernel<false, false, 1, true>), grid, dim3(NTHR), lds, (hipStream_t)stream, *a, LP, LDS_S);
        }
        PF_CHECK_LAUNCH();
        return 0;
    }
    switch (variant) {
        PF_NT_CASE(0, false, false, 1) PF_NT_CASE(1, false, true, 1) PF_NT_CASE(2, true, false, 1) PF_NT_CASE(3, true, true, 1)
        PF_NT_CASE(4, false, false, 2) PF_NT_CASE(5, false, true, 2) PF_NT_CASE(6, true, false, 2) PF_NT_CASE(7, true, true, 2)
    }
#undef PF_NT_CASE
    PF_CHECK_LAUNCH();
    return 0;
}
```

Before: 3.028 million res*step/s.

## Swizzle f16 LDS operand planes and stage bias/LN constants in shared memory

```diff
diff --git a/pepflowww_amd/csrc/common.h b/pepflowww_amd/csrc/common.h
--- a/pepflowww_amd/csrc/common.h
+++ b/pepflowww_amd/csrc/common.h
@@ -242,7 +242,7 @@
 __device__ __forceinline__ void gemm_split16(WSplit<WT, D, SP>& ws, const _Float16* Xh, const _Float16* Xl, int ldx,
                                              f32x4 (&am)[WT], f32x4 (&ac)[WT], int step0, int count) {
     const int lane = threadIdx.x & 63;
-    const int off = (lane & 15) * ldx + 8 * (lane >> 4);
+    const int off = (lane & 15) * ldx + 8 * ((lane >> 4) ^ ((lane >> 2) & 1));
     for (int base = 0; base < count; base += D) {
 #pragma unroll
         for (int u = 0; u < D; ++u) {
@@ -268,7 +268,7 @@
 __device__ __forceinline__ void gemm_split16r(WSplit<WT, D, SP>& ws, const _Float16* Xh, const _Float16* Xl, int ldx,
                                               f32x4 (&am)[RT][WT], f32x4 (&ac)[RT][WT], int step0, int count) {
     const int lane = threadIdx.x & 63;
-    const int off = (lane & 15) * ldx + 8 * (lane >> 4);
+    const int off = (lane & 15) * ldx + 8 * ((lane >> 4) ^ ((lane >> 2) & 1));
     for (int base = 0; base < count; base += D) {
 #pragma unroll
         for (int u = 0; u < D; ++u) {
diff --git a/pepflowww_amd/csrc/node_track.hip b/pepflowww_amd/csrc/node_track.hip
--- a/pepflowww_amd/csrc/node_track.hip
+++ b/pepflowww_amd/csrc/node_track.hip
@@ -19,7 +19,9 @@
 
 constexpr int TR = 16;
 constexpr int LDX = 132;
-constexpr int LDP = 136;
+constexpr int LDP = 144;
+constexpr int LDC = 256 + 16;
+__device__ __forceinline__ int pcol(int row, int col) { return col ^ ((row & 4) << 1); }
 constexpr int NTHR = 512;
 #ifndef PF_NT_MINW
 #define PF_NT_MINW 2
@@ -27,16 +29,24 @@
 
 struct Planes { _Float16* h; _Float16* l; };
 
-struct LnParams { float g[8], b[8]; };
-__device__ __forceinline__ void ln_load(LnParams& p, const float* __restrict__ g, const float* __restrict__ b) {
-    const int sub = threadIdx.x & 15;
-    const float4 g0 = *reinterpret_cast<const float4*>(g + 8 * sub), g1 = *reinterpret_cast<const float4*>(g + 8 * sub + 4);
-    const float4 b0 = *reinterpret_cast<const float4*>(b + 8 * sub), b1 = *reinterpret_cast<const float4*>(b + 8 * sub + 4);
-    p.g[0] = g0.x; p.g[1] = g0.y; p.g[2] = g0.z; p.g[3] = g0.w; p.g[4] = g1.x; p.g[5] = g1.y; p.g[6] = g1.z; p.g[7] = g1.w;
-    p.b[0] = b0.x; p.b[1] = b0.y; p.b[2] = b0.z; p.b[3] = b0.w; p.b[4] = b1.x; p.b[5] = b1.y; p.b[6] = b1.z; p.b[7] = b1.w;
+__device__ __forceinline__ const float* ct_pick(int i, const float* p0, const float* p1, const float* p2, const float* p3,
+                                                const float* p4, const float* p5, const float* p6, const float* p7) {
+    const float* p = p0;
+    p = i == 1 ? p1 : p; p = i == 2 ? p2 : p; p = i == 3 ? p3 : p; p = i == 4 ? p4 : p;
+    p = i == 5 ? p5 : p; p = i == 6 ? p6 : p; p = i == 7 ? p7 : p;
+    return p;
+}
+constexpr int CT_N1G = 0, CT_N1B = 128, CT_N2G = 256, CT_N2B = 384, CT_B1 = 512, CT_B2 = 640;
+constexpr int CT_IN = 768;
+constexpr int CT_NTG = 768, CT_NTB = 896, CT_POST = 1024, CT_T1 = 1152, CT_T2 = 1280, CT_T3 = 1408,
+              CT_PRE = 1536 , CT_INIT = 2048 , CT_BB = 2112 , CT_SIZE = 2120;
+constexpr int HT_LNG = 0, HT_LNB = 128, HT_OUT = 256, HT_IN = 384 , HT_SIZE = 768;
+__device__ __forceinline__ float4 ct_fetch(const float* pa, const float* pb) {
+    const int lane = threadIdx.x & 63;
+    return *reinterpret_cast<const float4*>((lane < 32 ? pa : pb) + 4 * (lane & 31));
 }
 template <int ROWS = 16, bool KFR = false>
-__device__ __forceinline__ void ln_tile(float* T, const LnParams& p, float mk, Planes out, int m0, int M, float* gout, _Float16* kf = nullptr, int i0 = 0) {
+__device__ __forceinline__ void ln_tile(float* T, const float* lg, const float* lb, float mk, Planes out, int m0, int M, float* gout, _Float16* kf = nullptr, int i0 = 0) {
     const int tid = threadIdx.x;
     if (tid < 16 * ROWS) {
         const int row = tid >> 4, sub = tid & 15, m = m0 + row;
@@ -46,6 +56,9 @@
             const float4 b = *reinterpret_cast<const float4*>(T + row * LDX + 8 * sub + 4);
             v[0] = a.x; v[1] = a.y; v[2] = a.z; v[3] = a.w; v[4] = b.x; v[5] = b.y; v[6] = b.z; v[7] = b.w;
         }
+        const float4 g0 = *reinterpret_cast<const float4*>(lg + 8 * sub), g1 = *reinterpret_cast<const float4*>(lg + 8 * sub + 4);
+        const float4 b0 = *reinterpret_cast<const float4*>(lb + 8 * sub), b1 = *reinterpret_cast<const float4*>(lb + 8 * sub + 4);
+        const float pg[8] = {g0.x, g0.y, g0.z, g0.w, g1.x, g1.y, g1.z, g1.w}, pb[8] = {b0.x, b0.y, b0.z, b0.w, b1.x, b1.y, b1.z, b1.w};
         float s = ((v[0] + v[1]) + (v[2] + v[3])) + ((v[4] + v[5]) + (v[6] + v[7]));
         s = row16_sum(s);
         const float mean = s / 128.f;
@@ -56,17 +69,18 @@
         const float rstd = rsqrtf(q / 128.f + 1e-5f);
         float y[8];
 #pragma unroll
-        for (int c = 0; c < 8; ++c) y[c] = ((v[c] - mean) * rstd * p.g[c] + p.b[c]) * mk;
+        for (int c = 0; c < 8; ++c) y[c] = ((v[c] - mean) * rstd * pg[c] + pb[c]) * mk;
         *reinterpret_cast<float4*>(T + row * LDX + 8 * sub) = make_float4(y[0], y[1], y[2], y[3]);
         *reinterpret_cast<float4*>(T + row * LDX + 8 * sub + 4) = make_float4(y[4], y[5], y[6], y[7]);
         half4 h0, l0, h1, l1;
         const float y0[4] = {y[0], y[1], y[2], y[3]}, y1[4] = {y[4], y[5], y[6], y[7]};
         split4(y0, h0, l0);
         split4(y1, h1, l1);
-        *reinterpret_cast<half4*>(out.h + row * LDP + 8 * sub) = h0;
-        *reinterpret_cast<half4*>(out.h + row * LDP + 8 * sub + 4) = h1;
-        *reinterpret_cast<half4*>(out.l + row * LDP + 8 * sub) = l0;
-        *reinterpret_cast<half4*>(out.l + row * LDP + 8 * sub + 4) = l1;
+        const int pc = row * LDP + pcol(row, 8 * sub);
+        *reinterpret_cast<half4*>(out.h + pc) = h0;
+        *reinterpret_cast<half4*>(out.h + pc + 4) = h1;
+        *reinterpret_cast<half4*>(out.l + pc) = l0;
+        *reinterpret_cast<half4*>(out.l + pc + 4) = l1;
         if (gout && m < M) {
             *reinterpret_cast<float4*>(gout + (size_t)m * 128 + 8 * sub) = make_float4(y[0], y[1], y[2], y[3]);
             *reinterpret_cast<float4*>(gout + (size_t)m * 128 + 8 * sub + 4) = make_float4(y[4], y[5], y[6], y[7]);
@@ -88,17 +102,18 @@
 __device__ __forceinline__ void put_planes(Planes p, int r, int n, const float (&v)[4]) {
     half4 hi, lo;
     split4(v, hi, lo);
-    *reinterpret_cast<half4*>(p.h + r * LDP + n) = hi;
-    *reinterpret_cast<half4*>(p.l + r * LDP + n) = lo;
+    *reinterpret_cast<half4*>(p.h + r * LDP + pcol(r, n)) = hi;
+    *reinterpret_cast<half4*>(p.l + r * LDP + pcol(r, n)) = lo;
 }
 
 template <bool SP, bool DUMP = false, bool PM = false>
 __global__ __launch_bounds__(NTHR, PF_NT_MINW) void node_head_kernel(pf_node_head_args a) {
     extern __shared__ __attribute__((aligned(16))) unsigned char smem_raw[];
-    constexpr int CK = 256, LDC = CK + 8;
+    constexpr int CK = 256;
     _Float16* Ch = reinterpret_cast<_Float16*>(smem_raw);
     float* X = reinterpret_cast<float*>(smem_raw + 2 * 2 * TR * LDC * sizeof(_Float16));
     Planes Xa = {reinterpret_cast<_Float16*>(X + TR * LDX), reinterpret_cast<_Float16*>(X + TR * LDX) + TR * LDP};
+    float* HT = reinterpret_cast<float*>(Xa.l + TR * LDP);
     const int tid = threadIdx.x, wave = tid >> 6, lane = tid & 63;
     const int r = lane & 15, g = lane >> 4;
     const int m0 = blockIdx.x * TR, M = a.rows;
@@ -109,12 +124,9 @@
     WSplit<1, 8, SP> ws;
     ws.init(a.w_out_f16, 128, PF_IPA_FEATS - C0 * 256, wave * 16);
     ws.prefetch();
-    LnParams lnp;
-    ln_load(lnp, a.ln_g, a.ln_b);
-    const float4 bias_out = *reinterpret_cast<const float4*>(a.b_out + n);
-    float4 bias_in[3];
-#pragma unroll
-    for (int wt = 0; wt < 3; ++wt) bias_in[wt] = *reinterpret_cast<const float4*>(a.b_in + wave * 48 + wt * 16 + 4 * g);
+    const int wu = __builtin_amdgcn_readfirstlane(wave);
+    const float4 ht0 = ct_fetch(ct_pick(wu, a.ln_g, a.b_out, a.b_in + 128, a.ln_g, a.ln_g, a.ln_g, a.ln_g, a.ln_g),
+                                ct_pick(wu, a.ln_b, a.b_in, a.b_in + 256, a.ln_g, a.ln_g, a.ln_g, a.ln_g, a.ln_g));
     const int mr = m0 + r;
     const int mrc = mr < M ? mr : M - 1;
     const float rmask_ld = a.mask[mrc];
@@ -138,8 +150,8 @@
             const float v[4] = {sv.x, sv.y, sv.z, sv.w};
             half4 hi, lo;
             split4(v, hi, lo);
-            *reinterpret_cast<half4*>(bh + srow * LDC + hlf * 128 + 4 * sc4) = hi;
-            *reinterpret_cast<half4*>(bl + srow * LDC + hlf * 128 + 4 * sc4) = lo;
+            *reinterpret_cast<half4*>(bh + srow * LDC + pcol(srow, hlf * 128 + 4 * sc4)) = hi;
+            *reinterpret_cast<half4*>(bl + srow * LDC + pcol(srow, hlf * 128 + 4 * sc4)) = lo;
         }
     };
     if constexpr (PM) {
@@ -150,6 +162,7 @@
         *reinterpret_cast<float4*>(X + srow * LDX + 4 * sc4) = add4(ev, od);
     }
     commit(C0);
+    if (tid < HT_SIZE / 4) *reinterpret_cast<float4*>(HT + 4 * tid) = ht0;
     __syncthreads();
     f32x4 am[1], ac[1];
     acc_zero1<1>(am, ac);
@@ -169,6 +182,7 @@
         float4 hs = make_float4(0.f, 0.f, 0.f, 0.f);
         if constexpr (PM) hs = *reinterpret_cast<const float4*>(X + r * LDX + n);
         auto lin = [&](int e, float h) { const float j = join(am[0], ac[0], e); if constexpr (PM) return j + h; else return j; };
+        const float4 bias_out = *reinterpret_cast<const float4*>(HT + HT_OUT + n);
         float4 y;
         y.x = (lin(0, hs.x) + bias_out.x) * rmask + rres.x;
         y.y = (lin(1, hs.y) + bias_out.y) * rmask + rres.y;
@@ -178,10 +192,13 @@
         if constexpr (DUMP) { if (mr < M) *reinterpret_cast<float4*>(a.dump_a0 + (size_t)mr * 128 + n) = y; }
     }
     __syncthreads();
-    ln_tile(X, lnp, 1.f, Xa, m0, M, a.s_ipa);
+    ln_tile(X, HT + HT_LNG, HT + HT_LNB, 1.f, Xa, m0, M, a.s_ipa);
     __syncthreads();
     f32x4 qm[3], qc[3];
     acc_zero1<3>(qm, qc);
+    float4 bias_in[3];
+#pragma unroll
+    for (int wt = 0; wt < 3; ++wt) bias_in[wt] = *reinterpret_cast<const float4*>(HT + HT_IN + wave * 48 + wt * 16 + 4 * g);
     gemm_split16(wq, Xa.h, Xa.l, LDP, qm, qc, 0, 4);
     if (mr < M) {
 #pragma unroll
@@ -198,10 +215,11 @@
 template <bool SP, bool PM = false>
 __global__ __launch_bounds__(NTHR, PF_NT_MINW) void node_head32_kernel(pf_node_head_args a) {
     extern __shared__ __attribute__((aligned(16))) unsigned char smem_raw[];
-    constexpr int CK = 256, LDC = CK + 8;
+    constexpr int CK = 256;
     _Float16* Ch = reinterpret_cast<_Float16*>(smem_raw);
     float* X = reinterpret_cast<float*>(smem_raw + 2 * 2 * TR2 * LDC * sizeof(_Float16));
     Planes Xa = {reinterpret_cast<_Float16*>(X + TR2 * LDX), reinterpret_cast<_Float16*>(X + TR2 * LDX) + TR2 * LDP};
+    float* HT = reinterpret_cast<float*>(Xa.l + TR2 * LDP);
     const int tid = threadIdx.x, wave = tid >> 6, lane = tid & 63;
     const int r = lane & 15, g = lane >> 4;
     int m0 = blockIdx.x * TR2, M = a.rows;
@@ -217,12 +235,9 @@
     WSplit<1, 8, SP> ws;
     ws.init(a.w_out_f16, 128, PF_IPA_FEATS - C0 * 256, wave * 16);
     ws.prefetch();
-    LnParams lnp;
-    ln_load(lnp, a.ln_g, a.ln_b);
-    const float4 bias_out = *reinterpret_cast<const float4*>(a.b_out + n);
-    float4 bias_in[3];
-#pragma unroll
-    for (int wt = 0; wt < 3; ++wt) bias_in[wt] = *reinterpret_cast<const float4*>(a.b_in + wave * 48 + wt * 16 + 4 * g);
+    const int wu = __builtin_amdgcn_readfirstlane(wave);
+    const float4 ht0 = ct_fetch(ct_pick(wu, a.ln_g, a.b_out, a.b_in + 128, a.ln_g, a.ln_g, a.ln_g, a.ln_g, a.ln_g),
+                                ct_pick(wu, a.ln_b, a.b_in, a.b_in + 256, a.ln_g, a.ln_g, a.ln_g, a.ln_g, a.ln_g));
     float rmask_ld[2];
     float4 rres_ld[2];
 #pragma unroll
@@ -252,8 +267,8 @@
             const float v[4] = {sv.x, sv.y, sv.z, sv.w};
             half4 hi, lo;
             split4(v, hi, lo);
-            *reinterpret_cast<half4*>(bh + row * LDC + 4 * c4) = hi;
-            *reinterpret_cast<half4*>(bl + row * LDC + 4 * c4) = lo;
+            *reinterpret_cast<half4*>(bh + row * LDC + pcol(row, 4 * c4)) = hi;
+            *reinterpret_cast<half4*>(bl + row * LDC + pcol(row, 4 * c4)) = lo;
         }
     };
     fetch(0, st[0]);
@@ -280,6 +295,7 @@
         }
     }
     commit(C0, st[C0 & 1]);
+    if (tid < HT_SIZE / 4) *reinterpret_cast<float4*>(HT + 4 * tid) = ht0;
     __syncthreads();
     f32x4 am[2][1], ac[2][1];
 #pragma unroll
@@ -295,6 +311,7 @@
     WSplit<3, 4, SP> wq;
     wq.init(a.w_in_f16, 384, 128, wave * 48);
     wq.prefetch();
+    const float4 bias_out = *reinterpret_cast<const float4*>(HT + HT_OUT + n);
 #pragma unroll
     for (int rt = 0; rt < 2; ++rt) {
         const int mr = m0 + rt * 16 + r;
@@ -311,11 +328,14 @@
         *reinterpret_cast<float4*>(X + (rt * 16 + r) * LDX + n) = y;
     }
     __syncthreads();
-    ln_tile<TR2>(X, lnp, 1.f, Xa, m0, M, a.s_ipa);
+    ln_tile<TR2>(X, HT + HT_LNG, HT + HT_LNB, 1.f, Xa, m0, M, a.s_ipa);
     __syncthreads();
     f32x4 qm[2][3], qc[2][3];
 #pragma unroll
     for (int rt = 0; rt < 2; ++rt) acc_zero1<3>(qm[rt], qc[rt]);
+    float4 bias_in[3];
+#pragma unroll
+    for (int wt = 0; wt < 3; ++wt) bias_in[wt] = *reinterpret_cast<const float4*>(HT + HT_IN + wave * 48 + wt * 16 + 4 * g);
     gemm_split16r<3, 4, SP, 2>(wq, Xa.h, Xa.l, LDP, qm, qc, 0, 4);
 #pragma unroll
     for (int rt = 0; rt < 2; ++rt) {
@@ -416,14 +436,19 @@
     WSplit<1, 4, SP> ws;
     ws.init(a.w_o_f16, 128, 128, wave * 16);
     ws.prefetch();
-    LnParams ln1, ln2, ln3;
-    ln_load(ln1, a.n1_g, a.n1_b);
-    ln_load(ln2, a.n2_g, a.n2_b);
-    if (LAST) ln_load(ln3, a.nt_g, a.nt_b);
-    const float4 bias_o = *reinterpret_cast<const float4*>(a.b_o + n), bias_1 = *reinterpret_cast<const float4*>(a.b_1 + n),
-                 bias_2 = *reinterpret_cast<const float4*>(a.b_2 + n);
-    float4 bias_post = z4, bias_t1 = z4, bias_t2 = z4, bias_t3 = z4, bias_bb = z4, bias_init = z4;
-    float4 bias_in[3] = {z4, z4, z4}, bias_pre[4] = {z4, z4, z4, z4};
+    const int wu = __builtin_amdgcn_readfirstlane(wave);
+    const float4 bias_o = *reinterpret_cast<const float4*>(a.b_o + n);
+    float4 ct0, ct1 = z4;
+    if constexpr (LAST) {
+        const float* pre = a.has_et ? a.b_pre + 256 * (wu & 1) : a.n1_g;
+        ct0 = ct_fetch(ct_pick(wu, a.n1_g, a.n2_g, a.b_1, a.nt_g, a.b_post, a.b_t2, pre, pre),
+                       ct_pick(wu, a.n1_b, a.n2_b, a.b_2, a.nt_b, a.b_t1, a.b_t3, a.has_et ? pre + 128 : pre, a.has_et ? pre + 128 : pre));
+        ct1 = *reinterpret_cast<const float4*>(a.has_et && tid < 16 ? a.b_init + 4 * tid : a.b_bb + (tid == 17 ? 4 : 0));
+    } else {
+        const float* bin = a.b_in_next;
+        ct0 = ct_fetch(ct_pick(wu, a.n1_g, a.n2_g, a.b_1, bin, bin + 256, bin, bin, bin),
+                       ct_pick(wu, a.n1_b, a.n2_b, a.b_2, bin + 128, bin + 256, bin, bin, bin));
+    }
     float4 rres_ld[RT], rsipa_ld[RT];
 #pragma unroll
     for (int rt = 0; rt < RT; ++rt) {
@@ -431,27 +456,9 @@
         rres_ld[rt] = *reinterpret_cast<const float4*>(a.resid + (size_t)mrc * 128 + n);
         rsipa_ld[rt] = LAST ? *reinterpret_cast<const float4*>(a.s_ipa + (size_t)mrc * 128 + n) : z4;
     }
-    float lnmask_ld = 1.f;
     const int lnrow = m0 + ((tid & (16 * TR - 1)) >> 4);
-    auto load_tail_consts = [&]() {
-        bias_post = *reinterpret_cast<const float4*>(a.b_post + n);
-        bias_t1 = *reinterpret_cast<const float4*>(a.b_t1 + n);
-        bias_t2 = *reinterpret_cast<const float4*>(a.b_t2 + n);
-        bias_t3 = *reinterpret_cast<const float4*>(a.b_t3 + n);
-        bias_bb = *reinterpret_cast<const float4*>(a.b_bb + 4 * (g & 1));
-        if (a.has_et) {
-            bias_init = *reinterpret_cast<const float4*>(a.b_init + (wave & 3) * 16 + 4 * g);
-#pragma unroll
-            for (int wt = 0; wt < 4; ++wt) bias_pre[wt] = *reinterpret_cast<const float4*>(a.b_pre + wave * 64 + wt * 16 + 4 * g);
-        }
-        lnmask_ld = a.mask[lnrow < M ? lnrow : M - 1];
-    };
-    if (LAST) {
-        if (RT == 1) load_tail_consts();
-    } else {
-#pragma unroll
-        for (int wt = 0; wt < 3; ++wt) bias_in[wt] = *reinterpret_cast<const float4*>(a.b_in_next + wave * 48 + wt * 16 + 4 * g);
-    }
+    const float lnmask_ld = LAST ? a.mask[lnrow < M ? lnrow : M - 1] : 1.f;
+    asm volatile("" ::: "memory");
 
     PROF(1);
     {
@@ -557,14 +564,18 @@
 #pragma unroll
             for (int e = 0; e < 4; ++e) {
                 const _Float16 hi = (_Float16)acc[rt][e];
-                Xa.h[(16 * rt + 4 * g + e) * LDP + col] = hi;
-                Xa.l[(16 * rt + 4 * g + e) * LDP + col] = (_Float16)((acc[rt][e] - (float)hi) * PF_LO_SCALE);
+                const int pc = (16 * rt + 4 * g + e) * LDP + pcol(4 * g + e, col);
+                Xa.h[pc] = hi;
+                Xa.l[pc] = (_Float16)((acc[rt][e] - (float)hi) * PF_LO_SCALE);
                 if constexpr (DUMP) { if (m0 + 16 * rt + 4 * g + e < M) a.dump[0][(size_t)(m0 + 16 * rt + 4 * g + e) * 128 + col] = acc[rt][e]; }
             }
     }
-    if (LAST && RT == 2) load_tail_consts();
     __syncthreads();
     PROF(4);
+    float* CT = S;
+    if (LAST || tid < (CT_IN + 384) / 4) *reinterpret_cast<float4*>(CT + 4 * tid) = ct0;
+    if (LAST && tid < 18) *reinterpret_cast<float4*>(CT + (tid < 16 ? CT_INIT + 4 * tid : CT_BB + 4 * (tid - 16))) = ct1;
+    auto cbias = [&](int off) { return *reinterpret_cast<const float4*>(CT + off); };
 
     f32x4 am[RT][1], ac[RT][1];
     auto zero = [&]() {
@@ -592,9 +603,10 @@
         dump4(a.dump[1], rt, v[0] + rres.x, v[1] + rres.y, v[2] + rres.z, v[3] + rres.w);
     }
     __syncthreads();
-    ln_tile<TR>(T1, ln1, 1.f, Xb, m0, M, DUMP ? a.dump[2] : nullptr);
+    ln_tile<TR>(T1, CT + CT_N1G, CT + CT_N1B, 1.f, Xb, m0, M, DUMP ? a.dump[2] : nullptr);
     __syncthreads();
     PROF(5);
+    const float4 bias_1 = cbias(CT_B1 + n);
     zero();
     gemm_split16r<1, 4, SP, RT>(ws, Xb.h, Xb.l, LDP, am, ac, 0, 4);
     ws.init(a.w_2_f16, 128, 128, wave * 16);
@@ -609,6 +621,7 @@
     }
     __syncthreads();
     PROF(6);
+    const float4 bias_2 = cbias(CT_B2 + n);
     zero();
     gemm_split16r<1, 4, SP, RT>(ws, Xa.h, Xa.l, LDP, am, ac, 0, 4);
     auto lin2_to_t0 = [&]() {
@@ -627,12 +640,15 @@
         wq.prefetch();
         lin2_to_t0();
         __syncthreads();
-        ln_tile<TR>(T0, ln2, 1.f, Xb, m0, M, a.v_out);
+        ln_tile<TR>(T0, CT + CT_N2G, CT + CT_N2B, 1.f, Xb, m0, M, a.v_out);
         __syncthreads();
         PROF(7);
         f32x4 qm[RT][3], qc[RT][3];
 #pragma unroll
         for (int rt = 0; rt < RT; ++rt) acc_zero1<3>(qm[rt], qc[rt]);
+        float4 bias_in[3];
+#pragma unroll
+        for (int wt = 0; wt < 3; ++wt) bias_in[wt] = cbias(CT_IN + wave * 48 + wt * 16 + 4 * g);
         gemm_split16r<3, 4, SP, RT>(wq, Xb.h, Xb.l, LDP, qm, qc, 0, 4);
 #pragma unroll
         for (int rt = 0; rt < RT; ++rt) {
@@ -663,9 +679,10 @@
             fmask = a.mask[m];
         }
         __syncthreads();
-        ln_tile<TR>(T0, ln2, 1.f, Xb, m0, M, DUMP ? a.dump[5] : nullptr);
+        ln_tile<TR>(T0, CT + CT_N2G, CT + CT_N2B, 1.f, Xb, m0, M, DUMP ? a.dump[5] : nullptr);
         __syncthreads();
         PROF(7);
+        const float4 bias_post = cbias(CT_POST + n);
         zero();
         gemm_split16r<1, 4, SP, RT>(ws, Xb.h, Xb.l, LDP, am, ac, 0, 4);
         ws.init(a.w_t1_f16, 128, 128, wave * 16);
@@ -682,6 +699,7 @@
         }
         __syncthreads();
         PROF(8);
+        const float4 bias_t1 = cbias(CT_T1 + n);
         zero();
         gemm_split16r<1, 4, SP, RT>(ws, Xa.h, Xa.l, LDP, am, ac, 0, 4);
         ws.init(a.w_t2_f16, 128, 128, wave * 16);
@@ -695,6 +713,7 @@
             dump4(a.dump[7], rt, v[0], v[1], v[2], v[3]);
         }
         __syncthreads();
+        const float4 bias_t2 = cbias(CT_T2 + n);
         zero();
         gemm_split16r<1, 4, SP, RT>(ws, Xb.h, Xb.l, LDP, am, ac, 0, 4);
         ws.init(a.w_t3_f16, 128, 128, wave * 16);
@@ -708,6 +727,7 @@
             dump4(a.dump[8], rt, v[0], v[1], v[2], v[3]);
         }
         __syncthreads();
+        const float4 bias_t3 = cbias(CT_T3 + n);
         zero();
         gemm_split16r<1, 4, SP, RT>(ws, Xa.h, Xa.l, LDP, am, ac, 0, 4);
         const bool do_bb = wave == 0, do_init = a.has_et && wave >= 4;
@@ -725,21 +745,22 @@
         }
         __syncthreads();
         _Float16* kfs = DUMP || !a.k_frag_s ? nullptr : reinterpret_cast<_Float16*>(a.k_frag_s) + (size_t)b * ((L + 15) >> 4) * (PF_KFRAG_TILE_B / 2);
-        ln_tile<TR, !DUMP>(T0, ln3, lnmask_ld * (lnrow < M ? 1.f : 0.f), Xb, m0, M, a.s_out, kfs, i0);
+        ln_tile<TR, !DUMP>(T0, CT + CT_NTG, CT + CT_NTB, lnmask_ld * (lnrow < M ? 1.f : 0.f), Xb, m0, M, a.s_out, kfs, i0);
         __syncthreads();
         PROF(9);
         if (do_bb || do_init) {
+            const float4 bias_bi = cbias(do_bb ? CT_BB + 4 * (g & 1) : CT_INIT + (wave & 3) * 16 + 4 * g);
             zero();
             gemm_split16r<1, 4, SP, RT>(ws, Xb.h, Xb.l, LDP, am, ac, 0, 4);
 #pragma unroll
             for (int rt = 0; rt < RT; ++rt) {
                 float v[4];
                 if (do_bb) {
-                    joined(rt, bias_bb, v);
+                    joined(rt, bias_bi, v);
                     if (g < 2) *reinterpret_cast<float4*>(U + (16 * rt + r) * 8 + 4 * g) = make_float4(v[0], v[1], v[2], v[3]);
                     if constexpr (DUMP) { if (g < 2 && mr[rt] < M) *reinterpret_cast<float4*>(a.dump[10] + (size_t)mr[rt] * 8 + 4 * g) = make_float4(v[0], v[1], v[2], v[3]); }
                 } else {
-                    joined(rt, bias_init, v);
+                    joined(rt, bias_bi, v);
                     put_planes(Xa, 16 * rt + r, (wave - 4) * 16 + 4 * g, v);
                 }
             }
@@ -761,6 +782,9 @@
             f32x4 pm[RT][4], pc[RT][4];
 #pragma unroll
             for (int rt = 0; rt < RT; ++rt) acc_zero1<4>(pm[rt], pc[rt]);
+            float4 bias_pre[4];
+#pragma unroll
+            for (int wt = 0; wt < 4; ++wt) bias_pre[wt] = cbias(CT_PRE + wave * 64 + wt * 16 + 4 * g);
             PROF(12);
             gemm_split16r<4, 2, SP, RT>(wp, Xa.h, Xa.l, LDP, pm, pc, 0, 2);
             PROF(13);
@@ -831,7 +855,7 @@
     }
 }
 
-constexpr int LDF = 640 + 8;
+constexpr int LDF = 640 + 16;
 template <bool SP>
 __global__ __launch_bounds__(NTHR) void input_mixer_kernel(pf_input_mixer_args a) {
     extern __shared__ __attribute__((aligned(16))) unsigned char smem_raw[];
@@ -891,8 +915,8 @@
         }
         half4 hi, lo;
         split4(v, hi, lo);
-        *reinterpret_cast<half4*>(Xf.h + row * LDF + 4 * c4) = hi;
-        *reinterpret_cast<half4*>(Xf.l + row * LDF + 4 * c4) = lo;
+        *reinterpret_cast<half4*>(Xf.h + row * LDF + pcol(row, 4 * c4)) = hi;
+        *reinterpret_cast<half4*>(Xf.l + row * LDF + pcol(row, 4 * c4)) = lo;
     }
     if (tid < TR && m0 + tid < M) {
         float R[9], q[4];
@@ -947,10 +971,11 @@
     if (!a || !a->feats || !a->s_in || !a->mask || !a->w_out_f16 || !a->b_out || !a->ln_g || !a->ln_b || !a->w_in_f16 ||
         !a->b_in || !a->s_ipa || !a->qkv || a->rows <= 0)
         return PF_E_BADARG;
-    const size_t lds = (size_t)2 * 2 * TR * 264 * sizeof(_Float16) + (size_t)TR * LDX * sizeof(float) +
-                       (size_t)2 * TR * LDP * sizeof(_Float16);
+    const size_t lds = (size_t)2 * 2 * TR * LDC * sizeof(_Float16) + (size_t)TR * LDX * sizeof(float) +
+                       (size_t)2 * TR * LDP * sizeof(_Float16) + HT_SIZE * sizeof(float);
     if (a->rows >= pf_cu_count() * TR2 && !a->dump_a0) {
-        const size_t lds2 = (size_t)2 * 2 * TR2 * 264 * sizeof(_Float16) + (size_t)TR2 * LDX * sizeof(float) + (size_t)2 * TR2 * LDP * sizeof(_Float16);
+        const size_t lds2 = (size_t)2 * 2 * TR2 * LDC * sizeof(_Float16) + (size_t)TR2 * LDX * sizeof(float) + (size_t)2 * TR2 * LDP * sizeof(_Float16) +
+                            HT_SIZE * sizeof(float);
         static PfOncePerDevice attr_set;
         if (attr_set.first()) {
             (void)hipFuncSetAttribute((const void*)node_head32_kernel<true>, hipFuncAttributeMaxDynamicSharedMemorySize, 160 * 1024);
@@ -1007,7 +1032,8 @@
     const int tiles16 = (a->L + 15) / 16;
     auto lds_of = [&](int rt) {
         const int tr = 16 * rt;
-        return ((size_t)2 * tr * LDX + tr * 8 + (size_t)tr * 4 * LDS_S) * sizeof(float) + (size_t)4 * tr * LDP * sizeof(_Float16);
+        const size_t s_floats = (size_t)tr * 4 * LDS_S > (size_t)CT_SIZE ? (size_t)tr * 4 * LDS_S : (size_t)CT_SIZE;
+        return ((size_t)2 * tr * LDX + tr * 8 + s_floats) * sizeof(float) + (size_t)4 * tr * LDP * sizeof(_Float16);
     };
     const int RTn = ((long)a->B * tiles16 > pf_cu_count() && a->L > 16 && !a->dump[0] && lds_of(2) <= (size_t)160 * 1024) ? 2 : 1;
     const int TRn = 16 * RTn;
```

Result: no change. 3.044 million res*step/s (median of 6 runs) (+0.5%).
